# KadAMRN/Data_Free_Quantization

Measured on AMD Instinct MI355X. Metric: weight-GB/s quantized (per-ch INT8 DFQ sweep) + top-1 delta, MobileNetV2, higher is better.
Workload: dtype f32

## Files before the change

data_free_quantization_amd/csrc/dfq_cle.hip:

```cpp
#include "dfq_cle_common.h"

#include <algorithm>
#include <atomic>
#include <chrono>
#include <cmath>
#include <cstdio>
#include <cstdlib>
#include <cstring>
#include <condition_variable>
#include <functional>
#include <list>
#include <memory>
#include <mutex>
#include <thread>
#include <unordered_map>
#include <new>
#include <numeric>
#include <vector>

using namespace dfq;

namespace dfq {

struct CleRel {
    float* w1;
    float* w2;
    float* b1;
    float* bnw;
    float* bnb;
    float* sacc;
    int64_t c1, len1, o2, i2, khw2, o2g;
    int64_t moff;
    int32_t sacc_init;
    int32_t vec1;
    int32_t vec2;
    int32_t fuse_next;
    int32_t dw_prev;
    int32_t w1_self;
    int32_t w2_self;
};

enum : int32_t { kRangeW1 = 0, kRangeW2Contig = 1, kRangeW2Tile = 2, kRangeReset = 3, kRangeResetW1 = 4 };
enum : int32_t { kApplyW1 = 0, kApplyW2Contig = 1, kApplyW2Tile = 2, kApplyChannels = 3, kApplyDwBoth = 4 };

struct CleTask {
    int32_t rel;
    int32_t kind;
    int64_t a, b;
    int64_t c0, c1;
};

struct CleLayer {
    float* w;
    float* snap;
    int64_t n;
    int64_t nt;
};

struct CleChunk {
    int32_t layer;
    int32_t t;
    int64_t c0;
    int64_t len;
};

struct CleState {
    double diff;
    double thr;
    int32_t iter_count;
    int32_t iters;
    int32_t done;
    int32_t count;
    int32_t max_iters;
    int32_t error;
};

constexpr int kCleW1RowsPerTask = 4;
constexpr int kCleW2ChansPerTask = 4;

__host__ __device__ inline int row_group_lanes(int64_t len) {
    if (len >= 64) return 64;
    int g = 1;
    while (g < len) g <<= 1;
    return g;
}
__host__ __device__ inline int64_t rows_per_task(int64_t len) { return 4 * (64 / row_group_lanes(len)); }

__device__ __forceinline__ float group_min(float v, int g) {
    for (int off = g >> 1; off >= 1; off >>= 1) v = fminf(v, __shfl_xor(v, off, 64));
    return v;
}
__device__ __forceinline__ float group_max(float v, int g) {
    for (int off = g >> 1; off >= 1; off >>= 1) v = fmaxf(v, __shfl_xor(v, off, 64));
    return v;
}
template <class F>
__device__ __forceinline__ void for_short_rows(int64_t a, int64_t b, int64_t len, F&& f) {
    const int lane = threadIdx.x & 63, wv = threadIdx.x >> 6;
    const int G = row_group_lanes(len), rpw = 64 / G;
    const int sub = lane / G, sl = lane % G;
    for (int64_t base = a + (int64_t)wv * rpw; base < b; base += (int64_t)(kThreads / 64) * rpw) {
        const int64_t c = base + sub;
        f(c, c < b, sl, G);
    }
}
constexpr int64_t kCleChansPerTask = 1024;
constexpr int64_t kCleW1SmallElems = 2048, kCleDwRowsMult = 1;

__device__ __forceinline__ void wave_range(const float* __restrict__ p_, int64_t n, bool vec, int lane, float& vmin,
                                           float& vmax) {
    const DFQ_GLOBAL float* __restrict__ p = (const DFQ_GLOBAL float*)p_;
    vmin = INFINITY;
    vmax = -INFINITY;
    if (vec) {
        const DFQ_GLOBAL f32x4* p4 = (const DFQ_GLOBAL f32x4*)p;
        const int64_t n4 = n >> 2;
        for (int64_t i = lane; i < n4; i += 4 * 64) {
            f32x4 v[4];
#pragma unroll
            for (int u = 0; u < 4; ++u)
                if (i + 64 * u < n4) v[u] = p4[i + 64 * u];
#pragma unroll
            for (int u = 0; u < 4; ++u)
                if (i + 64 * u < n4) {
                    vmin = fminf(vmin, fminf(fminf(v[u].x, v[u].y), fminf(v[u].z, v[u].w)));
                    vmax = fmaxf(vmax, fmaxf(fmaxf(v[u].x, v[u].y), fmaxf(v[u].z, v[u].w)));
                }
        }
    } else {
        for (int64_t i = lane; i < n; i += 4 * 64) {
            float v[4];
#pragma unroll
            for (int u = 0; u < 4; ++u)
                if (i + 64 * u < n) v[u] = p[i + 64 * u];
#pragma unroll
            for (int u = 0; u < 4; ++u)
                if (i + 64 * u < n) {
                    vmin = fminf(vmin, v[u]);
                    vmax = fmaxf(vmax, v[u]);
                }
        }
    }
    cle_wave_minmax(vmin, vmax);
}

template <class F>
__device__ __forceinline__ void wave_scale(float* __restrict__ p_, int64_t n, bool vec, int lane, F&& factor) {
    DFQ_GLOBAL float* __restrict__ p = (DFQ_GLOBAL float*)p_;
    float f = 0.f;
    bool have = false;
    if (vec) {
        DFQ_GLOBAL f32x4* p4 = (DFQ_GLOBAL f32x4*)p;
        const int64_t n4 = n >> 2;
        for (int64_t i = lane; i < n4; i += 4 * 64) {
            f32x4 v[4];
#pragma unroll
            for (int u = 0; u < 4; ++u)
                if (i + 64 * u < n4) v[u] = p4[i + 64 * u];
            if (!have) {
                f = factor();
                have = true;
            }
#pragma unroll
            for (int u = 0; u < 4; ++u)
                if (i + 64 * u < n4) {
                    v[u].x = v[u].x * f;
                    v[u].y = v[u].y * f;
                    v[u].z = v[u].z * f;
                    v[u].w = v[u].w * f;
                    p4[i + 64 * u] = v[u];
                }
        }
    } else {
        for (int64_t i = lane; i < n; i += 4 * 64) {
            float v[4];
#pragma unroll
            for (int u = 0; u < 4; ++u)
                if (i + 64 * u < n) v[u] = p[i + 64 * u];
            if (!have) {
                f = factor();
                have = true;
            }
#pragma unroll
            for (int u = 0; u < 4; ++u)
                if (i + 64 * u < n) p[i + 64 * u] = v[u] * f;
        }
    }
}

template <class F>
__device__ __forceinline__ void wave_scale_mm(float* __restrict__ p_, int64_t n, bool vec, int lane, float& vmin,
                                              float& vmax, F&& factor) {
    DFQ_GLOBAL float* __restrict__ p = (DFQ_GLOBAL float*)p_;
    vmin = INFINITY;
    vmax = -INFINITY;
    float f = 0.f;
    bool have = false;
    if (vec) {
        DFQ_GLOBAL f32x4* p4 = (DFQ_GLOBAL f32x4*)p;
        const int64_t n4 = n >> 2;
        for (int64_t i = lane; i < n4; i += 4 * 64) {
            f32x4 v[4];
#pragma unroll
            for (int u = 0; u < 4; ++u)
                if (i + 64 * u < n4) v[u] = p4[i + 64 * u];
            if (!have) {
                f = factor();
                have = true;
            }
#pragma unroll
            for (int u = 0; u < 4; ++u)
                if (i + 64 * u < n4) {
                    v[u].x = v[u].x * f;
                    v[u].y = v[u].y * f;
                    v[u].z = v[u].z * f;
                    v[u].w = v[u].w * f;
                    p4[i + 64 * u] = v[u];
                    vmin = fminf(vmin, fminf(fminf(v[u].x, v[u].y), fminf(v[u].z, v[u].w)));
                    vmax = fmaxf(vmax, fmaxf(fmaxf(v[u].x, v[u].y), fmaxf(v[u].z, v[u].w)));
                }
        }
    } else {
        for (int64_t i = lane; i < n; i += 4 * 64) {
            float v[4];
#pragma unroll
            for (int u = 0; u < 4; ++u)
                if (i + 64 * u < n) v[u] = p[i + 64 * u];
            if (!have) {
                f = factor();
                have = true;
            }
#pragma unroll
            for (int u = 0; u < 4; ++u)
                if (i + 64 * u < n) {
                    const float y = v[u] * f;
                    p[i + 64 * u] = y;
                    vmin = fminf(vmin, y);
                    vmax = fmaxf(vmax, y);
                }
        }
    }
    cle_wave_minmax(vmin, vmax);
}

template <class F>
__device__ __forceinline__ void wave_scale_range(float* __restrict__ p_, int64_t n, int lane, float& vmin, float& vmax,
                                                 F&& factor) {
    DFQ_GLOBAL float* __restrict__ p = (DFQ_GLOBAL float*)p_;
    vmin = INFINITY;
    vmax = -INFINITY;
    float f = 0.f;
    bool have = false;
    for (int64_t i = lane; i < n; i += 64) {
        const float x = p[i];
        if (!have) {
            f = factor();
            have = true;
        }
        const float y = x * f;
        p[i] = y;
        vmin = fminf(vmin, y);
        vmax = fmaxf(vmax, y);
    }
    cle_wave_minmax(vmin, vmax);
}

constexpr int kTileMaxKhw = 9;
#ifndef DFQ_CLE_POS_ROWS
#define DFQ_CLE_POS_ROWS 4
#endif
constexpr int kPosTileMaxRows = DFQ_CLE_POS_ROWS;

__device__ __forceinline__ bool tile_by_position(const CleRel& R, const CleTask& tk) {
    return R.khw2 > 1 && R.khw2 <= kTileMaxKhw && (tk.a / R.o2g) == ((tk.b - 1) / R.o2g);
}

__device__ void tile_range_by_position(const CleRel& R, const CleTask& tk, uint32_t* __restrict__ mn,
                                       uint32_t* __restrict__ mx, float* __restrict__ tl) {
    const int t = threadIdx.x;
    const int khw = (int)R.khw2;
    const int64_t rowlen = R.i2 * R.khw2;
    const int ncol = (int)(tk.c1 - tk.c0);
    const int npos = ncol * khw;
    const DFQ_GLOBAL float* base = (const DFQ_GLOBAL float*)(R.w2 + tk.c0 * R.khw2);
    float vmn[kTileMaxKhw], vmx[kTileMaxKhw];
#pragma unroll
    for (int m = 0; m < kTileMaxKhw; ++m) {
        vmn[m] = INFINITY;
        vmx[m] = -INFINITY;
    }
    for (int64_t o = tk.a; o < tk.b; ++o) {
        const DFQ_GLOBAL float* rp = base + o * rowlen;
        float v[kTileMaxKhw];
#pragma unroll
        for (int m = 0; m < kTileMaxKhw; ++m)
            if (m < khw && t + kThreads * m < npos) v[m] = rp[t + kThreads * m];
#pragma unroll
        for (int m = 0; m < kTileMaxKhw; ++m)
            if (m < khw && t + kThreads * m < npos) {
                vmn[m] = fminf(vmn[m], v[m]);
                vmx[m] = fmaxf(vmx[m], v[m]);
            }
    }
#pragma unroll
    for (int m = 0; m < kTileMaxKhw; ++m)
        if (m < khw && t + kThreads * m < npos) {
            tl[t + kThreads * m] = vmn[m];
            tl[kThreads * kTileMaxKhw + t + kThreads * m] = vmx[m];
        }
    __syncthreads();
    if (t < ncol) {
        float a = INFINITY, b = -INFINITY;
        for (int k = 0; k < khw; ++k) {
            a = fminf(a, tl[t * khw + k]);
            b = fmaxf(b, tl[kThreads * kTileMaxKhw + t * khw + k]);
        }
        const int64_t c = R.c1 + (tk.a / R.o2g) * R.i2 + tk.c0 + t;
        atomicMin(&mn[c], enc_ord(a));
        atomicMax(&mx[c], enc_ord(b));
    }
    __syncthreads();
}

__device__ __forceinline__ void cle_range_body(const CleRel* __restrict__ rels, const CleTask* __restrict__ tasks,
                                               int64_t t0, int64_t t1, uint32_t* __restrict__ rng, int64_t M, int par,
                                               int64_t blk, int64_t nblk, float* tl) {
    uint32_t* mins = rng + (int64_t)par * 2 * M;
    uint32_t* maxs = mins + M;
    uint32_t* omins = rng + (int64_t)(par ^ 1) * 2 * M;
    uint32_t* omaxs = omins + M;
    const int lane = threadIdx.x & 63;
    const int wv = threadIdx.x >> 6;
    for (int64_t t = t0 + blk; t < t1; t += nblk) {
        const CleTask tk = tasks[t];
        const CleRel& R = rels[tk.rel];
        uint32_t* mn = mins + R.moff;
        uint32_t* mx = maxs + R.moff;
        if (tk.kind == kRangeW1 && R.len1 < 64) {
            for_short_rows(tk.a, tk.b, R.len1, [&](int64_t c, bool act, int sl, int G) {
                float vmin = INFINITY, vmax = -INFINITY;
                if (act)
                    for (int64_t i = sl; i < R.len1; i += G) {
                        const float x = ((DFQ_GLOBAL float*)R.w1)[c * R.len1 + i];
                        vmin = fminf(vmin, x);
                        vmax = fmaxf(vmax, x);
                    }
                vmin = group_min(vmin, G);
                vmax = group_max(vmax, G);
                if (act && sl == 0) {
                    mn[c] = enc_ord(vmin);
                    mx[c] = enc_ord(vmax);
                }
            });
        } else if (tk.kind == kRangeW2Contig && R.o2g * R.khw2 < 64) {
            const int64_t seg = R.o2g * R.khw2;
            for_short_rows(tk.a, tk.b, seg, [&](int64_t c, bool act, int sl, int G) {
                float vmin = INFINITY, vmax = -INFINITY;
                if (act)
                    for (int64_t i = sl; i < seg; i += G) {
                        const float x = ((DFQ_GLOBAL float*)R.w2)[c * seg + i];
                        vmin = fminf(vmin, x);
                        vmax = fmaxf(vmax, x);
                    }
                vmin = group_min(vmin, G);
                vmax = group_max(vmax, G);
                if (act && sl == 0) {
                    mn[R.c1 + c] = enc_ord(vmin);
                    mx[R.c1 + c] = enc_ord(vmax);
                }
            });
        } else if (tk.kind == kRangeW1) {
            for (int64_t c = tk.a + wv; c < tk.b; c += kThreads / 64) {
                float vmin, vmax;
                wave_range(R.w1 + c * R.len1, R.len1, R.vec1, lane, vmin, vmax);
                if (lane == 0) {
                    mn[c] = enc_ord(vmin);
                    mx[c] = enc_ord(vmax);
                }
            }
        } else if (tk.kind == kRangeW2Contig) {
            const int64_t seg = R.o2g * R.khw2;
            for (int64_t c = tk.a + wv; c < tk.b; c += kThreads / 64) {
                float vmin, vmax;
                wave_range(R.w2 + c * seg, seg, R.vec2, lane, vmin, vmax);
                if (lane == 0) {
                    mn[R.c1 + c] = enc_ord(vmin);
                    mx[R.c1 + c] = enc_ord(vmax);
                }
            }
        } else if (tk.kind == kRangeW2Tile) {
            if (tile_by_position(R, tk)) {
                tile_range_by_position(R, tk, mn, mx, tl);
                continue;
            }
            const int64_t rowlen = R.i2 * R.khw2;
            const bool one_group = (tk.a / R.o2g) == ((tk.b - 1) / R.o2g);
            for (int64_t i = tk.c0 + threadIdx.x; i < tk.c1; i += kThreads) {
                float vmin = INFINITY, vmax = -INFINITY;
                if (one_group && R.khw2 == 1) {
                    float v[kColTileRows];
#pragma unroll
                    for (int j = 0; j < kColTileRows; ++j)
                        if (tk.a + j < tk.b) v[j] = ((DFQ_GLOBAL float*)R.w2)[(tk.a + j) * rowlen + i];
#pragma unroll
                    for (int j = 0; j < kColTileRows; ++j)
                        if (tk.a + j < tk.b) {
                            vmin = fminf(vmin, v[j]);
                            vmax = fmaxf(vmax, v[j]);
                        }
                    const int64_t c = R.c1 + (tk.a / R.o2g) * R.i2 + i;
                    atomicMin(&mn[c], enc_ord(vmin));
                    atomicMax(&mx[c], enc_ord(vmax));
                    continue;
                }
                int64_t g_prev = -1;
                for (int64_t o = tk.a; o < tk.b; ++o) {
                    const int64_t g = o / R.o2g;
                    if (g != g_prev && g_prev >= 0) {
                        atomicMin(&mn[R.c1 + g_prev * R.i2 + i], enc_ord(vmin));
                        atomicMax(&mx[R.c1 + g_prev * R.i2 + i], enc_ord(vmax));
                        vmin = INFINITY;
                        vmax = -INFINITY;
                    }
                    g_prev = g;
                    const DFQ_GLOBAL float* p = (const DFQ_GLOBAL float*)(R.w2 + o * rowlen + i * R.khw2);
                    for (int64_t k = 0; k < R.khw2; ++k) {
                        vmin = fminf(vmin, p[k]);
                        vmax = fmaxf(vmax, p[k]);
                    }
                }
                if (g_prev >= 0) {
                    atomicMin(&mn[R.c1 + g_prev * R.i2 + i], enc_ord(vmin));
                    atomicMax(&mx[R.c1 + g_prev * R.i2 + i], enc_ord(vmax));
                }
            }
        } else {
            const int64_t off = R.moff + (tk.kind == kRangeReset ? R.c1 : 0);
            for (int64_t c = tk.a + threadIdx.x; c < tk.b; c += kThreads) {
                omins[off + c] = 0xFFFFFFFFu;
                omaxs[off + c] = 0u;
            }
        }
    }
}

__global__ void __launch_bounds__(kThreads)
cle_loop_range_kernel(const CleRel* __restrict__ rels, const CleTask* __restrict__ tasks, int64_t t0, int64_t t1,
                      uint32_t* __restrict__ rng, int64_t M, const CleState* __restrict__ st, int next) {
    __shared__ float tl[2 * kThreads * kTileMaxKhw];
    if (st->done) return;
    cle_range_body(rels, tasks, t0, t1, rng, M, (st->iters + next) & 1, blockIdx.x, gridDim.x, tl);
}

__device__ __forceinline__ CleScale cle_rel_scale(const CleRel* __restrict__ rels, const CleRel& R,
                                                  const uint32_t* __restrict__ mins, const uint32_t* __restrict__ maxs,
                                                  int64_t c, int is_signed, float eps, double smin, double smax) {
    if (R.dw_prev < 0) return cle_scale(mins + R.moff, maxs + R.moff, R.c1, c, is_signed, eps, smin, smax);
    const CleRel& Q = rels[R.dw_prev];
    const CleScale q = cle_scale(mins + Q.moff, maxs + Q.moff, Q.c1, c, is_signed, eps, smin, smax);
    const float mn1 = dec_ord(mins[Q.moff + Q.c1 + c]) * q.inv;
    const float mx1 = dec_ord(maxs[Q.moff + Q.c1 + c]) * q.inv;
    return cle_scale_from(mn1, mx1, dec_ord(mins[R.moff + R.c1 + c]), dec_ord(maxs[R.moff + R.c1 + c]), is_signed, eps,
                          smin, smax);
}

struct CleApplyLds {
    float red[2][kThreads / 64][kColTileRows];
    float inv_s[kThreads];
    float inv_pos[kThreads * kTileMaxKhw];
    float rows[kColTileRows * kThreads];
};

#ifdef DFQ_DIAGNOSTICS
__device__ uint64_t* g_cle_tl = nullptr;
__device__ uint64_t* g_cle_tl2 = nullptr;
__device__ int64_t g_cle_tl2_a0 = -1;
constexpr int kCleTl2Fin = 8192;
#endif

template <bool POS = true>
__device__ __forceinline__ void cle_apply_body(const CleRel* __restrict__ rels, const CleTask* __restrict__ tasks,
                                               int64_t t0, int64_t t1, uint32_t* __restrict__ rng, int64_t M,
                                               int par, bool first_iter, int is_signed, float eps, double smin,
                                               double smax, int64_t blk, int64_t nblk, CleApplyLds& A,
                                               float* __restrict__ vsave = nullptr, int32_t* __restrict__ vtag = nullptr,
                                               int32_t iter = 0) {
    auto& red = A.red;
    float* rows = A.rows;
    float* inv_s = A.inv_s;
    float* inv_pos = A.inv_pos;
    uint32_t* mins = rng + (int64_t)par * 2 * M;
    uint32_t* maxs = mins + M;
    uint32_t* nmins = rng + (int64_t)(par ^ 1) * 2 * M;
    uint32_t* nmaxs = nmins + M;
    const int lane = threadIdx.x & 63;
    const int wv = threadIdx.x >> 6;
    for (int64_t t = t0 + blk; t < t1; t += nblk) {
#ifdef DFQ_DIAGNOSTICS
        const bool tl_on = g_cle_tl != nullptr;
        const uint64_t tl_start = tl_on ? __builtin_amdgcn_s_memrealtime() : 0;
        uint64_t tl_sub = 0;
#define DFQ_CLE_TL_MARK(k) \
        if (tl_on) tl_sub |= (1ull << 63) | (((__builtin_amdgcn_s_memrealtime() - tl_start) & 0xffffull) << (16 * (k)));
#else
#define DFQ_CLE_TL_MARK(k)
#endif
        const CleTask tk = tasks[t];
        const CleRel& R = rels[tk.rel];
        const uint32_t* mn = mins + R.moff;
        const uint32_t* mx = maxs + R.moff;
        if (tk.kind == kApplyW1 && R.len1 < 64) {
            for_short_rows(tk.a, tk.b, R.len1, [&](int64_t c, bool act, int sl, int G) {
                float y0 = INFINITY, y1 = -INFINITY;
                if (act && sl < R.len1) {
                    DFQ_GLOBAL float* p = (DFQ_GLOBAL float*)(R.w1 + c * R.len1 + sl);
                    const float x = *p;
                    const float y = x * cle_rel_scale(rels, R, mins, maxs, c, is_signed, eps, smin, smax).s;
                    *p = y;
                    y0 = y1 = y;
                }
                if (R.w1_self) {
                    y0 = group_min(y0, G);
                    y1 = group_max(y1, G);
                    if (act && sl == 0) {
                        nmins[R.moff + c] = enc_ord(y0);
                        nmaxs[R.moff + c] = enc_ord(y1);
                    }
                }
            });
        } else if (tk.kind == kApplyDwBoth && R.o2g * R.khw2 < 64) {
            const CleRel& N = rels[tk.c0];
            const int64_t seg = R.o2g * R.khw2;
            for_short_rows(tk.a, tk.b, seg, [&](int64_t c, bool act, int sl, int G) {
                float z0 = INFINITY, z1 = -INFINITY;
                if (act && sl < seg) {
                    DFQ_GLOBAL float* p = (DFQ_GLOBAL float*)(R.w2 + c * seg + sl);
                    const float x = *p;
                    const float inv = cle_rel_scale(rels, R, mins, maxs, c, is_signed, eps, smin, smax).inv;
                    const float sn = cle_rel_scale(rels, N, mins, maxs, c, is_signed, eps, smin, smax).s;
                    const float y = x * inv;
                    const float z = y * sn;
                    *p = z;
                    z0 = z1 = z;
                }
                if (R.w2_self) {
                    z0 = group_min(z0, G);
                    z1 = group_max(z1, G);
                    if (act && sl == 0) {
                        nmins[R.moff + R.c1 + c] = enc_ord(z0);
                        nmaxs[R.moff + R.c1 + c] = enc_ord(z1);
                    }
                }
            });
        } else if (tk.kind == kApplyW2Contig && R.o2g * R.khw2 < 64) {
            const int64_t seg = R.o2g * R.khw2;
            const bool fuse = R.fuse_next >= 0;
            for_short_rows(tk.a, tk.b, seg, [&](int64_t c, bool act, int sl, int G) {
                float vmin = INFINITY, vmax = -INFINITY;
                if (act && sl < seg) {
                    DFQ_GLOBAL float* p = (DFQ_GLOBAL float*)(R.w2 + c * seg + sl);
                    const float x = *p;
                    const float y = x * cle_rel_scale(rels, R, mins, maxs, c, is_signed, eps, smin, smax).inv;
                    *p = y;
                    vmin = vmax = y;
                }
                if (fuse) {
                    vmin = group_min(vmin, G);
                    vmax = group_max(vmax, G);
                    if (act && sl == 0) {
                        const int64_t off = rels[R.fuse_next].moff;
                        mins[off + c] = enc_ord(vmin);
                        maxs[off + c] = enc_ord(vmax);
                    }
                }
            });
        } else if (tk.kind == kApplyW1) {
            for (int64_t c = tk.a + wv; c < tk.b; c += kThreads / 64) {
                auto sc = [&] { return cle_rel_scale(rels, R, mins, maxs, c, is_signed, eps, smin, smax).s; };
                if (R.w1_self) {
                    float y0, y1;
                    wave_scale_mm(R.w1 + c * R.len1, R.len1, R.vec1, lane, y0, y1, sc);
                    if (lane == 0) {
                        nmins[R.moff + c] = enc_ord(y0);
                        nmaxs[R.moff + c] = enc_ord(y1);
                    }
                } else {
                    wave_scale(R.w1 + c * R.len1, R.len1, R.vec1, lane, sc);
                }
            }
        } else if (tk.kind == kApplyDwBoth) {
            const CleRel& N = rels[tk.c0];
            const int64_t seg = R.o2g * R.khw2;
            for (int64_t c = tk.a + wv; c < tk.b; c += kThreads / 64) {
                const float inv = cle_rel_scale(rels, R, mins, maxs, c, is_signed, eps, smin, smax).inv;
                const float sn = cle_rel_scale(rels, N, mins, maxs, c, is_signed, eps, smin, smax).s;
                DFQ_GLOBAL float* p = (DFQ_GLOBAL float*)(R.w2 + c * seg);
                float z0 = INFINITY, z1 = -INFINITY;
                for (int64_t i = lane; i < seg; i += 64) {
                    const float y = p[i] * inv;
                    const float z = y * sn;
                    p[i] = z;
                    z0 = fminf(z0, z);
                    z1 = fmaxf(z1, z);
                }
                if (R.w2_self) {
                    cle_wave_minmax(z0, z1);
                    if (lane == 0) {
                        nmins[R.moff + R.c1 + c] = enc_ord(z0);
                        nmaxs[R.moff + R.c1 + c] = enc_ord(z1);
                    }
                }
            }
        } else if (tk.kind == kApplyW2Contig) {
            const int64_t seg = R.o2g * R.khw2;
            for (int64_t c = tk.a + wv; c < tk.b; c += kThreads / 64) {
                auto inv = [&] { return cle_rel_scale(rels, R, mins, maxs, c, is_signed, eps, smin, smax).inv; };
                if (R.fuse_next >= 0) {
                    float vmin, vmax;
                    wave_scale_range(R.w2 + c * seg, seg, lane, vmin, vmax, inv);
                    if (lane == 0) {
                        const int64_t off = rels[R.fuse_next].moff;
                        mins[off + c] = enc_ord(vmin);
                        maxs[off + c] = enc_ord(vmax);
                    }
                } else {
                    wave_scale(R.w2 + c * seg, seg, R.vec2, lane, inv);
                }
            }
        } else if (POS && tk.kind == kApplyW2Tile && tile_by_position(R, tk) && tk.b - tk.a <= kPosTileMaxRows) {
            const int t = threadIdx.x;
            const int khw = (int)R.khw2;
            const int64_t rowlen = R.i2 * R.khw2;
            const int ncol = (int)(tk.c1 - tk.c0);
            const int npos = ncol * khw;
            DFQ_GLOBAL float* base = (DFQ_GLOBAL float*)(R.w2 + tk.c0 * R.khw2);
            const bool fuse = R.fuse_next >= 0;
            if (t < ncol)
                inv_s[t] = cle_rel_scale(rels, R, mins, maxs, (tk.a / R.o2g) * R.i2 + tk.c0 + t, is_signed, eps, smin, smax).inv;
            __syncthreads();
            DFQ_CLE_TL_MARK(0)
            for (int q = t; q < npos; q += kThreads) inv_pos[q] = inv_s[q / khw];
            __syncthreads();
            DFQ_CLE_TL_MARK(1)
            float v[kPosTileMaxRows][kTileMaxKhw];
#pragma unroll
            for (int r = 0; r < kPosTileMaxRows; ++r) {
                const DFQ_GLOBAL float* rb = base + (tk.a + r) * rowlen;
#pragma unroll
                for (int m = 0; m < kTileMaxKhw; ++m)
                    if (tk.a + r < tk.b && m < khw && t + kThreads * m < npos) v[r][m] = rb[t + kThreads * m];
            }
#pragma unroll
            for (int r = 0; r < kPosTileMaxRows; ++r) {
                if (tk.a + r >= tk.b) break;
                DFQ_GLOBAL float* rp = base + (tk.a + r) * rowlen;
                float lo = INFINITY, hi = -INFINITY;
#pragma unroll
                for (int m = 0; m < kTileMaxKhw; ++m)
                    if (m < khw && t + kThreads * m < npos) {
                        const float y = v[r][m] * inv_pos[t + kThreads * m];
                        rp[t + kThreads * m] = y;
                        lo = fminf(lo, y);
                        hi = fmaxf(hi, y);
                    }
                if (fuse) {
                    cle_wave_minmax(lo, hi);
                    if (lane == 0) {
                        red[0][wv][r] = lo;
                        red[1][wv][r] = hi;
                    }
                }
            }
            __syncthreads();
            DFQ_CLE_TL_MARK(2)
            if (fuse && t < tk.b - tk.a) {
                float a = red[0][0][t], b = red[1][0][t];
                for (int w = 1; w < kThreads / 64; ++w) {
                    a = fminf(a, red[0][w][t]);
                    b = fmaxf(b, red[1][w][t]);
                }
                const int64_t off = rels[R.fuse_next].moff + tk.a + t;
                atomicMin(&mins[off], enc_ord(a));
                atomicMax(&maxs[off], enc_ord(b));
            }
            __syncthreads();
        } else if (tk.kind == kApplyW2Tile && R.fuse_next >= 0) {
            const int64_t rowlen = R.i2 * R.khw2;
            const int64_t i = tk.c0 + threadIdx.x;
            const bool act = i < tk.c1;
            const bool one_group = (tk.a / R.o2g) == ((tk.b - 1) / R.o2g);
            const int nr = (int)(tk.b - tk.a);
            if (one_group && R.khw2 == 1) {
                float v[kColTileRows];
#pragma unroll
                for (int j = 0; j < kColTileRows; ++j)
                    if (act && j < nr) v[j] = ((DFQ_GLOBAL float*)R.w2)[(tk.a + j) * rowlen + i];
                const float inv =
                    act ? cle_rel_scale(rels, R, mins, maxs, (tk.a / R.o2g) * R.i2 + i, is_signed, eps, smin, smax).inv : 0.f;
#pragma unroll
                for (int j = 0; j < kColTileRows; ++j) {
                    if (j < nr) {
                        float y = __builtin_nanf("");
                        if (act) {
                            y = v[j] * inv;
                            ((DFQ_GLOBAL float*)R.w2)[(tk.a + j) * rowlen + i] = y;
                        }
                        rows[j * kThreads + threadIdx.x] = y;
                    }
                    if (j == 0) {
                        DFQ_CLE_TL_MARK(0)
                    }
                }
                DFQ_CLE_TL_MARK(1)
                block_lds_sync();
                const int r = threadIdx.x >> 4, sg = threadIdx.x & 15;
                float lo = INFINITY, hi = -INFINITY;
                if (r < nr) {
                    const float4* q = reinterpret_cast<const float4*>(rows + r * kThreads + sg * 16);
#pragma unroll
                    for (int u = 0; u < 4; ++u) {
                        const float4 x = q[u];
                        lo = fminf(lo, fminf(fminf(x.x, x.y), fminf(x.z, x.w)));
                        hi = fmaxf(hi, fmaxf(fmaxf(x.x, x.y), fmaxf(x.z, x.w)));
                    }
                }
                lo = fminf(lo, dpp_f(lo, 0xB1));
                hi = fmaxf(hi, dpp_f(hi, 0xB1));
                lo = fminf(lo, dpp_f(lo, 0x4E));
                hi = fmaxf(hi, dpp_f(hi, 0x4E));
                lo = fminf(lo, dpp_f(lo, 0x141));
                hi = fmaxf(hi, dpp_f(hi, 0x141));
                lo = fminf(lo, dpp_f(lo, 0x140));
                hi = fmaxf(hi, dpp_f(hi, 0x140));
                DFQ_CLE_TL_MARK(2)
                if (sg == 0 && r < nr) {
                    const int64_t off = rels[R.fuse_next].moff + tk.a + r;
                    atomicMin(&mins[off], enc_ord(lo));
                    atomicMax(&maxs[off], enc_ord(hi));
                }
            } else {
                int64_t g_prev = -1;
                float inv = 0.f;
                for (int j = 0; j < nr; ++j) {
                    const int64_t o = tk.a + j;
                    float lo = INFINITY, hi = -INFINITY;
                    if (act) {
                        const int64_t g = o / R.o2g;
                        if (g != g_prev) {
                            inv = cle_rel_scale(rels, R, mins, maxs, g * R.i2 + i, is_signed, eps, smin, smax).inv;
                            g_prev = g;
                        }
                        DFQ_GLOBAL float* p = (DFQ_GLOBAL float*)(R.w2 + o * rowlen + i * R.khw2);
                        for (int64_t k = 0; k < R.khw2; ++k) {
                            const float y = p[k] * inv;
                            p[k] = y;
                            lo = fminf(lo, y);
                            hi = fmaxf(hi, y);
                        }
                    }
                    float a = lo, b = hi;
                    cle_wave_minmax(a, b);
                    if (lane == 0) {
                        red[0][wv][j] = a;
                        red[1][wv][j] = b;
                    }
                }
                __syncthreads();
                if (threadIdx.x < tk.b - tk.a) {
                    const int j = threadIdx.x;
                    float a = red[0][0][j], b = red[1][0][j];
                    for (int w = 1; w < kThreads / 64; ++w) {
                        a = fminf(a, red[0][w][j]);
                        b = fmaxf(b, red[1][w][j]);
                    }
                    const int64_t off = rels[R.fuse_next].moff + tk.a + j;
                    atomicMin(&mins[off], enc_ord(a));
                    atomicMax(&maxs[off], enc_ord(b));
                }
            }
            __syncthreads();
        } else if (tk.kind == kApplyW2Tile) {
            const int64_t rowlen = R.i2 * R.khw2;
            const bool one_group = (tk.a / R.o2g) == ((tk.b - 1) / R.o2g);
            for (int64_t i = tk.c0 + threadIdx.x; i < tk.c1; i += kThreads) {
                if (one_group && R.khw2 == 1) {
                    float v[kColTileRows];
#pragma unroll
                    for (int j = 0; j < kColTileRows; ++j)
                        if (tk.a + j < tk.b) v[j] = ((DFQ_GLOBAL float*)R.w2)[(tk.a + j) * rowlen + i];
                    const float inv = cle_rel_scale(rels, R, mins, maxs, (tk.a / R.o2g) * R.i2 + i, is_signed, eps, smin,
                                                smax).inv;
                    ((DFQ_GLOBAL float*)R.w2)[tk.a * rowlen + i] = v[0] * inv;
                    DFQ_CLE_TL_MARK(0)
#pragma unroll
                    for (int j = 1; j < kColTileRows; ++j)
                        if (tk.a + j < tk.b) ((DFQ_GLOBAL float*)R.w2)[(tk.a + j) * rowlen + i] = v[j] * inv;
                    DFQ_CLE_TL_MARK(1)
                    continue;
                }
                int64_t g_prev = -1;
                float inv = 0.f;
                for (int64_t o = tk.a; o < tk.b; ++o) {
                    const int64_t g = o / R.o2g;
                    if (g != g_prev) {
                        inv = cle_rel_scale(rels, R, mins, maxs, g * R.i2 + i, is_signed, eps, smin, smax).inv;
                        g_prev = g;
                    }
                    DFQ_GLOBAL float* p = (DFQ_GLOBAL float*)(R.w2 + o * rowlen + i * R.khw2);
                    for (int64_t k = 0; k < R.khw2; ++k) p[k] = p[k] * inv;
                }
            }
        } else {
            if (vtag && threadIdx.x == 0) vtag[t] = iter;
            for (int64_t c = tk.a + threadIdx.x; c < tk.b; c += kThreads) {
                const CleScale cs = cle_rel_scale(rels, R, mins, maxs, c, is_signed, eps, smin, smax);
                if (vsave) {
                    float* v = vsave + 2 * R.moff;
                    if (R.b1) v[c] = R.b1[c];
                    if (R.bnw) v[R.c1 + c] = R.bnw[c];
                    if (R.bnb) v[2 * R.c1 + c] = R.bnb[c];
                    if (R.sacc) v[3 * R.c1 + c] = R.sacc[c];
                }
                if (R.b1) R.b1[c] = R.b1[c] * cs.s;
                if (R.bnw) R.bnw[c] = R.bnw[c] * cs.s;
                if (R.bnb) R.bnb[c] = R.bnb[c] * cs.s;
                if (R.sacc) R.sacc[c] = (R.sacc_init && first_iter) ? cs.s : R.sacc[c] * cs.s;
            }
        }
#ifdef DFQ_DIAGNOSTICS
        if (tl_on) {
            __syncthreads();
            if (threadIdx.x == 0) {
                uint32_t hw, xcc;
                asm volatile("s_getreg_b32 %0, hwreg(HW_REG_HW_ID)" : "=s"(hw));
                asm volatile("s_getreg_b32 %0, hwreg(HW_REG_XCC_ID)" : "=s"(xcc));
                uint64_t* r = g_cle_tl + 4 * t;
                r[0] = tl_start;
                r[1] = __builtin_amdgcn_s_memrealtime();
                r[2] = tl_sub ? tl_sub : (((uint64_t)xcc << 32) | hw);
                r[3] = (uint64_t)tk.kind | ((uint64_t)tk.rel << 8) | ((uint64_t)(tk.b - tk.a) << 24);
            }
        }
#endif
    }
}

constexpr int kCleTile = 8192;
constexpr int kCleTailWords = 64;

struct CleUnit {
    int32_t chunk;
    int32_t tile;
};

__global__ void __launch_bounds__(kThreads)
cle_loop_init_kernel(const CleLayer* __restrict__ layers, const CleChunk* __restrict__ chunks, int64_t nchunks,
                     const CleUnit* __restrict__ units, int64_t nunits, uint32_t* __restrict__ rng, int64_t M,
                     float* __restrict__ part, int64_t npart, uint32_t* __restrict__ cnt, int64_t ncnt,
                     int32_t* __restrict__ vtag, int64_t nvtag, CleState* __restrict__ st, CleState init) {
    const int64_t gt = (int64_t)blockIdx.x * kThreads + threadIdx.x, gs = (int64_t)gridDim.x * kThreads;
    for (int64_t i = gt; i < 4 * M; i += gs) rng[i] = ((i / M) & 1) ? 0u : 0xFFFFFFFFu;
    for (int64_t i = gt; i < npart; i += gs) part[i] = 0.f;
    for (int64_t i = gt; i < ncnt; i += gs) cnt[i] = 0u;
    for (int64_t i = gt; i < nvtag; i += gs) vtag[i] = -1;
    if (gt == 0) *st = init;
    for (int64_t u = blockIdx.x; u < nunits; u += gridDim.x) {
        const CleUnit un = units[u];
        const CleChunk ch = chunks[un.chunk];
        const CleLayer Ly = layers[ch.layer];
        const int64_t nb1 = (ch.len / 32) / 256;
        const int64_t e0 = (int64_t)un.tile * 8192;
        const int64_t e1 = un.tile < nb1 ? e0 + 8192 : ch.len;
        for (int64_t i = e0 + threadIdx.x; i < e1; i += kThreads) Ly.snap[ch.c0 + i] = Ly.w[ch.c0 + i];
    }
    if (blockIdx.x == 0)
        for (int64_t k = 0; k < nchunks; ++k) {
            const CleChunk ch = chunks[k];
            if (ch.len >= 8) continue;
            const CleLayer Ly = layers[ch.layer];
            for (int64_t i = threadIdx.x; i < ch.len; i += kThreads) Ly.snap[ch.c0 + i] = Ly.w[ch.c0 + i];
        }
}


struct CleNoUnitHook {
    __device__ void operator()(const CleUnit&, const CleChunk&, int64_t) const {}
};

template <class Hook = CleNoUnitHook>
__device__ __forceinline__ void cle_tiles_body(const CleLayer* __restrict__ layers, const CleChunk* __restrict__ chunks,
                                               const int64_t* __restrict__ b1off, const CleUnit* __restrict__ units,
                                               int64_t nunits, float* __restrict__ b1buf, float* __restrict__ tailbuf,
                                               int64_t blk, int64_t nblk, float* d, float* b0, Hook hook = Hook()) {
    const int tid = threadIdx.x;
    for (int64_t u = blk; u < nunits; u += nblk) {
        const CleUnit un = units[u];
        const CleChunk ch = chunks[un.chunk];
        const CleLayer Ly = layers[ch.layer];
        const DFQ_GLOBAL float* __restrict__ w = (const DFQ_GLOBAL float*)(Ly.w + ch.c0);
        DFQ_GLOBAL float* __restrict__ sn = (DFQ_GLOBAL float*)(Ly.snap + ch.c0);
        const int64_t len = ch.len, sz = len / 32, vs = len / 8;
        const int64_t nb1 = sz / 256;
        const bool full = un.tile < nb1;
        const int64_t e0 = (int64_t)un.tile * kCleTile;
        const int64_t cnt = full ? kCleTile : len - e0;
        if (full) {
            float xs[2][16], ys[2][16];
#pragma unroll
            for (int h = 0; h < 2; ++h) {
                const int q = tid + h * kThreads;
                const int64_t base = e0 + 32 * (16 * (q >> 5)) + (q & 31);
#pragma unroll
                for (int j = 0; j < 16; ++j) {
                    xs[h][j] = w[base + 32 * j];
                    ys[h][j] = sn[base + 32 * j];
                }
            }
#pragma unroll
            for (int h = 0; h < 2; ++h) {
                const int q = tid + h * kThreads;
                const int64_t base = e0 + 32 * (16 * (q >> 5)) + (q & 31);
                float a = 0.f;
#pragma unroll
                for (int j = 0; j < 16; ++j) {
                    a += fabsf(xs[h][j] - ys[h][j]);
                    sn[base + 32 * j] = xs[h][j];
                }
                b0[q] = a;
            }
            __syncthreads();
            if (tid < 32) {
                float a = 0.f;
#pragma unroll
                for (int m = 0; m < 16; ++m) a += b0[m * 32 + tid];
                st_coh(b1buf + b1off[un.chunk] + (int64_t)un.tile * 32 + tid, a);
            }
        } else {
            for (int64_t e = tid; e < cnt; e += 8 * kThreads) {
                float x[8], y[8];
#pragma unroll
                for (int u = 0; u < 8; ++u)
                    if (e + u * kThreads < cnt) {
                        x[u] = w[e0 + e + u * kThreads];
                        y[u] = sn[e0 + e + u * kThreads];
                    }
#pragma unroll
                for (int u = 0; u < 8; ++u)
                    if (e + u * kThreads < cnt) {
                        d[e + u * kThreads] = fabsf(x[u] - y[u]);
                        sn[e0 + e + u * kThreads] = x[u];
                    }
            }
            __syncthreads();
            const int64_t ni = sz - nb1 * 256;
            const int64_t rem_b0 = ni / 16, tail0 = ni % 16;
            float* tb = tailbuf + (int64_t)un.chunk * kCleTailWords;
            if (tid < 32) {
                float a1p = 0.f;
                for (int64_t m = 0; m < rem_b0; ++m) {
                    float a = 0.f;
                    for (int j = 0; j < 16; ++j) a += d[32 * (16 * m + j) + tid];
                    a1p += a;
                }
                float a0t = 0.f;
                for (int64_t j = 0; j < tail0; ++j) a0t += d[32 * (16 * rem_b0 + j) + tid];
                float p = a0t;
                p += a1p;
                st_coh(tb + tid, p);
            } else if (tid < 64) {
                const int t = tid - 32;
                const int64_t nv = vs - 4 * sz;
                if (t < 24 && t < nv * 8) st_coh(tb + 32 + t, d[8 * (4 * sz) + t - e0]);
                if (t < 8 && t < len - 8 * vs) st_coh(tb + 56 + t, d[8 * vs + t - e0]);
            }
        }
        __syncthreads();
        hook(un, ch, nb1);
    }
}

constexpr int kCleTilesLds = kCleTile + kCleTailWords + 512;
constexpr int kCleRangeLds = 2 * kThreads * kTileMaxKhw;

template <class LdB1, class LdTb>
__device__ __forceinline__ float cle_chunk_sum_with(const CleChunk& ch, LdB1&& b1, LdTb&& tb, int lane) {
    const int64_t len = ch.len;
    const int64_t sz = len / 32, vs = len / 8;
    const int64_t nb1 = sz / 256, nb2 = nb1 / 16, rem_b1 = nb1 % 16;
    float fa = 0.f;
    float p = 0.f;
    if (lane < 32) {
        float a3 = 0.f;
        for (int64_t r = 0; r < nb2; ++r) {
            float b2 = 0.f;
            for (int q = 0; q < 16; ++q) b2 += b1((r * 16 + q) * 32 + lane);
            a3 += b2;
        }
        float a2p = 0.f;
        for (int64_t q = 0; q < rem_b1; ++q) a2p += b1((nb2 * 16 + q) * 32 + lane);
        p = tb(lane);
        p += a2p;
        p += a3;
    }
    auto ps = [&](int s) { return rl_f(p, s); };
    for (int64_t e = 0; e < len - 8 * vs; ++e) fa += tb(56 + e);
    const int64_t nv = vs - 4 * sz;
    for (int l = 0; l < 8; ++l) {
        float p0 = ps(l);
        for (int64_t v = 0; v < nv; ++v) p0 += tb(32 + v * 8 + l);
        p0 += ps(l + 8);
        p0 += ps(l + 16);
        p0 += ps(l + 24);
        fa += p0;
    }
    return fa;
}

__device__ __forceinline__ float cle_chunk_sum(const CleChunk& ch, const float* b1, const float* tb, int lane) {
    const DFQ_GLOBAL float* g1 = (const DFQ_GLOBAL float*)b1;
    const DFQ_GLOBAL float* gt = (const DFQ_GLOBAL float*)tb;
    return cle_chunk_sum_with(ch, [g1](int64_t i) { return ld_coh(g1 + i); }, [gt](int64_t i) { return ld_coh(gt + i); },
                              lane);
}

__device__ __forceinline__ float cle_tiny_chunk_sum(const CleLayer* __restrict__ layers, const CleChunk& ch) {
    const CleLayer Ly = layers[ch.layer];
    float* w = Ly.w + ch.c0;
    float* sn = Ly.snap + ch.c0;
    return aten_inner_sum([&](int64_t e) {
        const float x = w[e];
        const float dd = fabsf(x - sn[e]);
        sn[e] = x;
        return dd;
    }, ch.len);
}

template <class P>
__device__ __forceinline__ double np_pairwise_leaf(P x, int64_t n) {
    if (n < 8) {
        double res = 0.;
        for (int64_t i = 0; i < n; ++i) res += x[i];
        return res;
    }
    double r[8];
#pragma unroll
    for (int j = 0; j < 8; ++j) r[j] = x[j];
    int64_t i;
    for (i = 8; i < n - (n % 8); i += 8)
#pragma unroll
        for (int j = 0; j < 8; ++j) r[j] += x[i + j];
    double res = ((r[0] + r[1]) + (r[2] + r[3])) + ((r[4] + r[5]) + (r[6] + r[7]));
    for (; i < n; ++i) res += x[i];
    return res;
}

struct NpFrame {
    int64_t o, n;
    int64_t state;
};
constexpr int kNpFrames = 48;
constexpr int kNpStackFloats = kNpFrames * (int)(sizeof(NpFrame) + sizeof(double)) / 4;
template <class P>
__device__ double np_pairwise(P a, int64_t n, float* stack) {
    if (n <= 128) return 0. + np_pairwise_leaf(a, n);
    NpFrame* fr = reinterpret_cast<NpFrame*>(stack);
    double* acc = reinterpret_cast<double*>(fr + kNpFrames);
    int fp = 0, ap = 0;
    fr[fp++] = {0, n, 0};
    while (fp > 0) {
        NpFrame& f = fr[fp - 1];
        if (f.n <= 128) {
            acc[ap++] = np_pairwise_leaf(a + f.o, f.n);
            --fp;
        } else if (f.state == 0) {
            int64_t n2 = f.n / 2;
            n2 -= n2 % 8;
            f.state = 1;
            const NpFrame left{f.o, n2, 0}, right{f.o + n2, f.n - n2, 0};
            fr[fp++] = right;
            fr[fp++] = left;
        } else {
            const double right = acc[--ap];
            const double left = acc[--ap];
            acc[ap++] = left + right;
            --fp;
        }
    }
    return 0. + acc[0];
}

template <bool kLeafOnly = false, bool kCoherent = false>
__device__ __forceinline__ void cle_final_body(const CleLayer* __restrict__ layers, int32_t nl,
                                               const float* __restrict__ part, int32_t S, double* __restrict__ means,
                                               double* __restrict__ hist, CleState* __restrict__ st, double* sm,
                                               float* part_lds = nullptr, float* np_stack = nullptr,
                                               uint32_t* hflag = nullptr) {
#ifdef DFQ_DIAGNOSTICS
    uint64_t* tlm = (kCoherent && threadIdx.x == 0 && g_cle_tl2) ? g_cle_tl2 + 4 * kCleTl2Fin : nullptr;
#endif
    constexpr int kStateWords = (int)(sizeof(CleState) / 4);
    static_assert(sizeof(CleState) % 4 == 0, "CleState: whole 4-B words");
    const int64_t nps = (int64_t)nl * (S + 2);
    DFQ_LDS float* pls = (DFQ_LDS float*)part_lds;
    if (part_lds) {
        for (int64_t i = threadIdx.x; i < nps + kStateWords; i += blockDim.x) {
            const DFQ_GLOBAL float* src = (const DFQ_GLOBAL float*)(i < nps ? part + i
                                                                           : reinterpret_cast<const float*>(st) + (i - nps));
            pls[i] = kCoherent ? ld_coh(src) : *src;
        }
        __syncthreads();
    }
#ifdef DFQ_DIAGNOSTICS
    if (tlm) tlm[2] = __builtin_amdgcn_s_memrealtime();
#endif
    DFQ_LDS double* ms = (DFQ_LDS double*)sm;
    DFQ_GLOBAL double* mg = (DFQ_GLOBAL double*)means;
    const bool m_lds = nl <= 1024;
    double* m = m_lds ? sm : means;
    for (int l = threadIdx.x; l < nl; l += blockDim.x) {
        const float* pl = (part_lds ? part_lds : part) + (int64_t)l * S;
        auto ld = [&](int64_t e) { return (part_lds || !kCoherent) ? pl[e] : ld_coh(pl + e); };
        const float* lm = part_lds ? part_lds + (int64_t)nl * S + 2 * l : nullptr;
        const bool serial = lm ? lm[1] != 0.f : layers[l].nt == 1;
        const float sum = serial ? 0.f + (0.f + ld(0)) : 0.f + aten_inner_sum([&](int64_t e) { return ld(e); }, S);
        m[l] = (double)(sum / (lm ? lm[0] : (float)layers[l].n));
    }
    __syncthreads();
#ifdef DFQ_DIAGNOSTICS
    if (tlm) tlm[3] = __builtin_amdgcn_s_memrealtime();
#endif
    if (threadIdx.x == 0) {
        CleState s0;
        if (part_lds) {
            __builtin_memcpy(&s0, part_lds + nps, sizeof(CleState));
        } else {
            s0 = *st;
        }
        double dt = 0.0;
        if constexpr (kLeafOnly) {
            dt = nl > 0 ? 0. + (m_lds ? np_pairwise_leaf(ms, nl) : np_pairwise_leaf(mg, nl)) : 0.0;
        } else {
            dt = nl > 0 ? (m_lds ? np_pairwise(ms, nl, np_stack) : np_pairwise(mg, nl, np_stack)) : 0.0;
        }
        const int it = s0.iters;
        hist[it] = dt;
        int ic = s0.iter_count;
        double diff = s0.diff;
        if (fabs(diff - dt) > 1e-9) {
            ic = 0;
            diff = dt;
        } else {
            ic += 1;
        }
        const bool cont = (diff > s0.thr) && (ic < s0.count);
        const int done = (!cont || it + 1 >= s0.max_iters) ? 1 : 0;
        st->iters = it + 1;
        st->iter_count = ic;
        st->diff = diff;
        st->done = done;
        if (hflag)
            __hip_atomic_store(hflag, ((uint32_t)(it + 1) << 1) | (uint32_t)done, __ATOMIC_RELAXED,
                               __HIP_MEMORY_SCOPE_SYSTEM);
    }
}

__device__ __forceinline__ bool handoff_arrive(uint32_t* c, uint32_t target) {
    return __hip_atomic_fetch_add(c, 1u, __ATOMIC_RELAXED, __HIP_MEMORY_SCOPE_AGENT) == target;
}

__host__ __device__ inline int64_t cle_stop_blocks(int64_t nchunks) {
    return nchunks > 0 ? (nchunks + kThreads / 64 - 1) / (kThreads / 64) : 1;
}

struct CleFin {
    uint32_t* cnt;
    float* part;
    double* means;
    double* hist;
    int64_t nchunks, nbig;
    int32_t S, nl;
    int32_t last;
    uint32_t* hflag;
    int32_t stop_arrival;
};

static_assert(kCleTilesLds - kCleTile >= kNpStackFloats, "np_pairwise's frame stack after the tile area");
union CleStepLds {
    CleApplyLds apply;
    float tiles[kCleTilesLds > kCleRangeLds ? kCleTilesLds : kCleRangeLds];
};

constexpr bool kCleTilesFirst = true;
#ifdef DFQ_DIAGNOSTICS
__device__ int g_cle_tiles_first = kCleTilesFirst ? 1 : 0;
#endif

template <bool POS>
#ifndef DFQ_CLE_POS_WAVES
#define DFQ_CLE_POS_WAVES 1
#endif
__global__ void __launch_bounds__(kThreads) __attribute__((amdgpu_waves_per_eu(POS ? DFQ_CLE_POS_WAVES : 4)))
cle_loop_step_kernel(const CleRel* __restrict__ rels, const CleTask* __restrict__ atasks, int64_t a0, int64_t a1,
                     int64_t nab, uint32_t* __restrict__ rng, int64_t M, int is_signed, float eps, double smin,
                     double smax, const CleLayer* __restrict__ layers, const CleChunk* __restrict__ chunks,
                     const int64_t* __restrict__ b1off, const CleUnit* __restrict__ units, int64_t uo, int64_t nuo,
                     int64_t nto, int64_t up, int64_t nup, int64_t ntp, float* __restrict__ b1buf,
                     float* __restrict__ tailbuf, const CleTask* __restrict__ rtasks, int64_t ro, int64_t nro_t,
                     int64_t nro, int64_t rp, int64_t nrp_t, int64_t nrp, CleFin F, CleState* __restrict__ st,
                     int32_t g, float* __restrict__ vsave, int32_t* __restrict__ vtag, int32_t stop_it) {
    __shared__ CleStepLds L;
    __shared__ int flag;
    if (st->done) return;
    int64_t blk = blockIdx.x;
#ifdef DFQ_DIAGNOSTICS
    const bool tiles_first = g_cle_tiles_first != 0;
#else
    constexpr bool tiles_first = kCleTilesFirst;
#endif
    const int64_t nstop = stop_it >= 0 ? cle_stop_blocks(F.nchunks) : 0;
    if (tiles_first) {
        const int64_t ns = nab + nstop, ntl = nto + ntp;
        if (blk < ntl) blk += ns;
        else if (blk < ntl + ns) blk -= ntl;
    }
    if (blk < nab) {
        cle_apply_body<POS>(rels, atasks, a0, a1, rng, M, g & 1, g == 0, is_signed, eps, smin, smax, blk, nab, L.apply,
                            vsave, vtag, g);
        return;
    }
    blk -= nab;
#ifdef DFQ_DIAGNOSTICS
    const bool tl2 = g_cle_tl2 != nullptr && blk < kCleTl2Fin && (g_cle_tl2_a0 < 0 || (a0 == g_cle_tl2_a0 && nab > 0));
    const uint64_t tl2_start = tl2 ? __builtin_amdgcn_s_memrealtime() : 0;
    auto tl2_rec = [&](int role) {
        if (tl2 && threadIdx.x == 0) {
            uint64_t* r = g_cle_tl2 + 4 * blk;
            r[0] = tl2_start;
            r[1] = __builtin_amdgcn_s_memrealtime();
            r[2] = (uint64_t)role;
        }
    };
#else
    auto tl2_rec = [](int) {};
#endif
    float* lds = L.tiles;
    auto finish = [&]() {
#ifdef DFQ_DIAGNOSTICS
        const uint64_t tf0 = __builtin_amdgcn_s_memrealtime();
#endif
        if (threadIdx.x == 0 && F.nchunks > F.nbig)
            for (int64_t k = 0; k < F.nchunks; ++k) {
                const CleChunk c2 = chunks[k];
                if (c2.len < 8) st_coh(F.part + (int64_t)c2.layer * F.S + c2.t, 0.f + cle_tiny_chunk_sum(layers, c2));
            }
        asm volatile("s_waitcnt vmcnt(0)" ::: "memory");
        __syncthreads();
        const bool stage_part = (int64_t)F.nl * (F.S + 2) + (int64_t)(sizeof(CleState) / 4) + 2048 <= kCleTile;
        if (F.nl <= 128)
            cle_final_body<true, true>(layers, F.nl, F.part, F.S, F.means, F.hist, st, reinterpret_cast<double*>(lds),
                                       stage_part ? lds + 2048 : nullptr, nullptr, F.hflag);
        else
            cle_final_body<false, true>(layers, F.nl, F.part, F.S, F.means, F.hist, st,
                                        reinterpret_cast<double*>(lds), stage_part ? lds + 2048 : nullptr,
                                        lds + kCleTile, F.hflag);
#ifdef DFQ_DIAGNOSTICS
        if (tl2 && threadIdx.x == 0) {
            uint64_t* r = g_cle_tl2 + 4 * kCleTl2Fin;
            r[0] = tf0;
            r[1] = __builtin_amdgcn_s_memrealtime();
        }
#endif
    };
    if (stop_it >= 0) {
        if (blk < nstop) {
            const int64_t c = blk * (kThreads / 64) + (threadIdx.x >> 6);
            if (c < F.nchunks) {
                const CleChunk ch = chunks[c];
                if (ch.len >= 8) {
                    const float fa = cle_chunk_sum(ch, b1buf + b1off[c], tailbuf + c * kCleTailWords, threadIdx.x & 63);
                    if ((threadIdx.x & 63) == 0) st_coh(F.part + (int64_t)ch.layer * F.S + ch.t, 0.f + fa);
                }
            }
            asm volatile("s_waitcnt vmcnt(0)" ::: "memory");
            __syncthreads();
            if (threadIdx.x == 0)
                flag = handoff_arrive(F.cnt + F.nchunks, ((uint32_t)stop_it + 1u) * (uint32_t)nstop - 1u);
            __syncthreads();
            if (flag) finish();
            return;
        }
        blk -= nstop;
    }
    const int64_t ntiles = nto + ntp;
    if (blk >= ntiles) {
        blk -= ntiles;
        const bool own = blk < nro;
        const int64_t b = own ? blk : blk - nro;
        cle_range_body(rels, rtasks, own ? ro : rp, (own ? ro : rp) + (own ? nro_t : nrp_t), rng, M,
                       own ? (g + 1) & 1 : g & 1, b, own ? nro : nrp, L.tiles);
        tl2_rec(2);
        return;
    }
    const bool own = blk < nto;
    const int32_t it = own ? g : g - 1;
    const int64_t tb = own ? blk : blk - nto;
    const int64_t tnb = own ? nto : ntp;
    const uint32_t round = (uint32_t)it + 1u;
    auto arrive = [&](uint32_t* c, uint32_t members) -> bool {
        asm volatile("s_waitcnt vmcnt(0)" ::: "memory");
        __syncthreads();
        if (threadIdx.x == 0) flag = handoff_arrive(c, round * members - 1u);
        __syncthreads();
        return flag != 0;
    };
    if (F.nbig == 0) {
        if (own && tb == 0 && F.last) finish();
        return;
    }
    const uint32_t fin_members = (uint32_t)F.nbig;
    auto hook = [&](const CleUnit& un, const CleChunk& ch, int64_t nb1) {
        if (!arrive(F.cnt + un.chunk, (uint32_t)(nb1 + 1))) return;
        {
            const float* gb1 = b1buf + b1off[un.chunk];
            const float* gtb = tailbuf + (int64_t)un.chunk * kCleTailWords;
            const int64_t nw = 32 * nb1;
            const bool staged = nw + kCleTailWords <= kCleTile;
            if (staged) {
                DFQ_LDS float* ll = (DFQ_LDS float*)lds;
                const DFQ_GLOBAL float* g1 = (const DFQ_GLOBAL float*)gb1;
                for (int64_t i = threadIdx.x; i < nw; i += kThreads) ll[i] = ld_coh(g1 + i);
                if (threadIdx.x < kCleTailWords) ll[nw + threadIdx.x] = ld_coh((const DFQ_GLOBAL float*)gtb + threadIdx.x);
            }
            __syncthreads();
            if (threadIdx.x < 64) {
                const float fa = staged ? cle_chunk_sum_with(ch, [&](int64_t i) { return lds[i]; },
                                                             [&](int64_t i) { return lds[nw + i]; }, threadIdx.x)
                                        : cle_chunk_sum(ch, gb1, gtb, threadIdx.x);
                if (threadIdx.x == 0) st_coh(F.part + (int64_t)ch.layer * F.S + ch.t, 0.f + fa);
            }
        }
        if (F.stop_arrival && arrive(F.cnt + F.nchunks, fin_members)) finish();
    };
    if (F.stop_arrival)
        cle_tiles_body<decltype(hook)>(layers, chunks, b1off, units + (own ? uo : up), own ? nuo : nup, b1buf, tailbuf,
                                       tb, tnb, lds, lds + kCleTile + kCleTailWords, hook);
    else
        cle_tiles_body(layers, chunks, b1off, units + (own ? uo : up), own ? nuo : nup, b1buf, tailbuf, tb, tnb, lds,
                       lds + kCleTile + kCleTailWords);
#ifdef DFQ_DIAGNOSTICS
    if (tl2) {
        const CleUnit un0 = units[(own ? uo : up) + tb];
        tl2_rec(un0.tile >= (chunks[un0.chunk].len / 32) / 256 ? 3 : 1);
    }
#else
    tl2_rec(1);
#endif
}

__global__ void __launch_bounds__(kThreads)
cle_loop_rollback_kernel(const CleLayer* __restrict__ layers, int32_t nl, const CleRel* __restrict__ rels,
                         const CleTask* __restrict__ atasks, int64_t n_at, const float* __restrict__ vsave,
                         const int32_t* __restrict__ vtag, const CleState* __restrict__ st) {
    const int32_t A = st->iters;
    const int64_t gt = (int64_t)blockIdx.x * kThreads + threadIdx.x, gs = (int64_t)gridDim.x * kThreads;
    for (int32_t l = 0; l < nl; ++l) {
        const CleLayer Ly = layers[l];
        for (int64_t i = gt; i < Ly.n; i += gs) Ly.w[i] = Ly.snap[i];
    }
    for (int64_t t = blockIdx.x; t < n_at; t += gridDim.x) {
        const CleTask tk = atasks[t];
        if (tk.kind != kApplyChannels || vtag[t] != A) continue;
        const CleRel& R = rels[tk.rel];
        const float* v = vsave + 2 * R.moff;
        for (int64_t c = tk.a + threadIdx.x; c < tk.b; c += kThreads) {
            if (R.b1) R.b1[c] = v[c];
            if (R.bnw) R.bnw[c] = v[R.c1 + c];
            if (R.bnb) R.bnb[c] = v[2 * R.c1 + c];
            if (R.sacc) R.sacc[c] = v[3 * R.c1 + c];
        }
    }
}

}

constexpr int32_t kCleHistCap = 1025;

struct dfq_cle_plan {
    CleRel* d_rels = nullptr;
    CleTask* d_rtasks = nullptr;
    CleTask* d_atasks = nullptr;
    CleLayer* d_layers = nullptr;
    CleChunk* d_chunks = nullptr;
    uint32_t* d_rng = nullptr;
    float* d_part = nullptr;
    int32_t slots = 8;
    double* d_means = nullptr;
    double* d_hist = nullptr;
    double* d_hist_tables = nullptr;
    CleState* d_state = nullptr;
    CleState* h_state = nullptr;
    uint32_t* d_flag = nullptr;
    uint64_t* d_sig = nullptr;
    uint64_t gen = 0;
    hipStream_t st = nullptr;
    std::vector<int64_t> rstep, astep;
    std::vector<char> step_pos;
    int64_t M = 0, nchunks = 0;
    int32_t nl = 0, chains = 0, steps = 0;
    bool fused = false;
    CleUnit* d_units = nullptr;
    int64_t* d_b1off = nullptr;
    float* d_b1 = nullptr;
    float* d_tail = nullptr;
    int64_t nunits = 0;
    double smin = 1e-8, smax = 1e8;
    int32_t is_signed = 0;
    float eps = 0.f;
    void* d_tables = nullptr;
    bool pooled = false;
    void* d_snap_owned = nullptr;
    uint32_t* d_cnt = nullptr;
    int64_t nbig = 0;
    int64_t ri0 = 0, ri1 = 0;
    std::vector<int64_t> uoffs, roffs;
    int32_t nlaunch = 0;
    int32_t stop_off = -1;
    bool lagged = false;
    float* d_vsave = nullptr;
    int32_t* d_vtag = nullptr;
    int64_t n_at = 0;
    int dev = 0;
    struct CleAsync* async = nullptr;
    bool abandoned = false;
    int64_t bytes[3] = {0, 0, 0};
    bool timed = false;
    float loop_ms = -1.f;
    int32_t launched = 0;
#ifdef DFQ_DIAGNOSTICS
    std::vector<CleRel> h_rels;
    std::vector<CleTask> h_atasks;
#endif
};

static bool cle_timing() {
    static const bool on = ab_env("DFQ_CLE_TIMING") != nullptr;
    return on;
}
static double now_us() {
    return std::chrono::duration<double, std::micro>(std::chrono::steady_clock::now().time_since_epoch()).count();
}

struct CleDeviceCtx {
    std::mutex mu;
    hipStream_t st = nullptr;
    CleState* h_state = nullptr;
    uint32_t* h_flag = nullptr;
    uint32_t* d_flag = nullptr;
    char* d_pool = nullptr;
    size_t pool_cap = 0;
    char* h_pool = nullptr;
    size_t hpool_cap = 0;
    bool pool_busy = false;
    uint64_t pool_struct = 0;
    hipEvent_t pool_ev = nullptr;
    double* d_hist = nullptr;
    int64_t hist_cap = 0;
    double* h_hist = nullptr;
    int64_t h_hist_cap = 0;
    void* sig = nullptr;
    int sig_state = 0;
    uint64_t gen = 0;
    struct dfq_cle_plan* pending = nullptr;
    hipEvent_t in_ev = nullptr;
    struct CleWorker* worker = nullptr;
};
static CleDeviceCtx& cle_device_ctx(int dev) {
    static CleDeviceCtx ctx[64];
    return ctx[dev & 63];
}
static hipError_t cle_ctx_ready(CleDeviceCtx& ctx) {
    hipError_t e = hipSuccess;
    if (!ctx.st) {
        int least = 0, greatest = 0;
        e = hipDeviceGetStreamPriorityRange(&least, &greatest);
        if (e == hipSuccess) e = hipStreamCreateWithPriority(&ctx.st, hipStreamNonBlocking, greatest);
    }
    if (e == hipSuccess && !ctx.h_state) e = hipHostMalloc(&ctx.h_state, sizeof(CleState));
    if (e == hipSuccess && !ctx.h_flag) {
        e = hipHostMalloc(&ctx.h_flag, 64, hipHostMallocMapped | hipHostMallocCoherent);
        if (e == hipSuccess) e = hipHostGetDevicePointer(reinterpret_cast<void**>(&ctx.d_flag), ctx.h_flag, 0);
    }
    if (e == hipSuccess && !ctx.pool_ev) e = hipEventCreateWithFlags(&ctx.pool_ev, hipEventDisableTiming);
    if (e == hipSuccess && !ctx.in_ev) e = hipEventCreateWithFlags(&ctx.in_ev, hipEventDisableTiming);
    return e;
}

static void cle_plan_free(dfq_cle_plan* p) {
    const double t0 = now_us();
    if (p->pooled) {
        CleDeviceCtx& ctx = cle_device_ctx(p->dev);
        std::lock_guard<std::mutex> lock(ctx.mu);
        ctx.pool_busy = false;
    } else {
        (void)hipFree(p->d_tables);
    }
    (void)hipFree(p->d_snap_owned);
    if (cle_timing()) fprintf(stderr, "DFQ_CLE_TIMING free: %.1f us\n", now_us() - t0);
    delete p;
}

static int64_t snap_bytes(int64_t n) { return ceil_div(n * (int64_t)sizeof(float), (int64_t)256) * 256; }

struct TableLayout {
    int64_t total = 0;
    template <typename T>
    int64_t add(int64_t count) {
        const int64_t off = total;
        total += ceil_div((int64_t)sizeof(T) * std::max<int64_t>(count, 1), (int64_t)256) * 256;
        return off;
    }
};

extern "C" int64_t dfq_cle_plan_ws_bytes(const int64_t* target_n, int32_t n_targets) {
    if (n_targets < 0 || (n_targets > 0 && !target_n)) return -1;
    int64_t b = 0;
    for (int32_t l = 0; l < n_targets; ++l) {
        if (target_n[l] < 0) return -1;
        b += snap_bytes(target_n[l]);
    }
    return b;
}

struct CleStructure {
    std::vector<CleRel> R;
    int64_t M = 0;
    int32_t chains = 0, steps = 0;
    bool fused = false;
    std::vector<CleTask> rt, at;
    std::vector<int64_t> rstep, astep;
    int64_t ri0 = 0, ri1 = 0;
    std::vector<CleLayer> layers;
    std::vector<CleChunk> chunks;
    std::vector<CleUnit> units;
    std::vector<int64_t> b1off;
    int64_t nb1_total = 0;
    std::vector<int64_t> uoffs, roffs;
    int32_t nlaunch = 0, stop_off = -1;
    bool lagged = false;
    double t_chains = 0, t_tasks = 0, t_chunks = 0, t_place = 0;
    int64_t bytes_rescale = 0, bytes_metric = 0, bytes_range = 0;
    uint64_t id = 0;
};
static std::atomic<uint64_t> g_struct_ids{0};

static int cle_build_structure(std::vector<CleRel> R, int64_t M, int32_t n_rel, float* const* targets,
                               const int64_t* target_n, int32_t n_targets, int32_t ref_threads, CleStructure& S) {
    const double tp1 = now_us();
    std::vector<int32_t> parent(n_rel);
    std::iota(parent.begin(), parent.end(), 0);
    auto find = [&](int32_t x) {
        while (parent[x] != x) x = parent[x] = parent[parent[x]];
        return x;
    };
    for (int32_t a = 0; a < n_rel; ++a) {
        const void* pa[5] = {R[a].w1, R[a].w2, R[a].b1, R[a].bnw, R[a].bnb};
        for (int32_t b = 0; b < a; ++b) {
            const void* pb[5] = {R[b].w1, R[b].w2, R[b].b1, R[b].bnw, R[b].bnb};
            bool share = false;
            for (int i = 0; i < 5 && !share; ++i)
                for (int j = 0; j < 5 && !share; ++j) share = pa[i] && pa[i] == pb[j];
            if (share) parent[find(a)] = find(b);
        }
    }
    std::vector<int32_t> step_of(n_rel), comp_len(n_rel, 0);
    int32_t chains = 0, steps = 0;
    for (int32_t r = 0; r < n_rel; ++r) {
        const int32_t c = find(r);
        if (comp_len[c] == 0) ++chains;
        step_of[r] = comp_len[c]++;
        steps = std::max(steps, step_of[r] + 1);
    }
    std::vector<int32_t> w1_src(n_rel, -1);
    bool fused = true;
    {
        const char* fe = ab_env("DFQ_CLE_FUSED");
        if (fe && fe[0] == '0') fused = false;
        std::vector<std::vector<int32_t>> chain_of(n_rel);
        for (int32_t r = 0; r < n_rel; ++r) chain_of[find(r)].push_back(r);
        for (const auto& L : chain_of) {
            for (size_t j = 0; j < L.size() && fused; ++j) {
                const CleRel& cr = R[L[j]];
                for (size_t i = 0; i < j && fused; ++i) {
                    const CleRel& cq = R[L[i]];
                    if (cq.w1 == cr.w2 || cq.w2 == cr.w2) fused = false;
                    if (cq.w1 == cr.w1 || cq.w2 == cr.w1) {
                        const bool ok = i + 1 == j && cq.w2 == cr.w1 && cq.w1 != cr.w1 && w1_src[L[j]] < 0 &&
                                        (cq.i2 > 1 || cq.o2g == 1) && cr.c1 == cq.o2 && cr.len1 == cq.i2 * cq.khw2;
                        if (ok) w1_src[L[j]] = L[i];
                        else fused = false;
                    }
                }
            }
        }
        if (fused)
            for (int32_t r = 0; r < n_rel; ++r)
                if (w1_src[r] >= 0) R[w1_src[r]].fuse_next = r;
    }
    std::vector<int32_t> dw_next(n_rel, -1);
    if (fused) {
        for (int32_t r = 0; r < n_rel; ++r) {
            const int32_t q = w1_src[r];
            if (q < 0 || R[q].dw_prev >= 0 || dw_next[q] >= 0) continue;
            const CleRel& cq = R[q];
            const CleRel& cr = R[r];
            const bool dw = cq.i2 == 1 && cq.o2g == 1 && cq.o2 == cq.c1 && cr.c1 == cq.o2 && cr.len1 == cq.khw2;
            if (!dw) continue;
            R[r].dw_prev = q;
            R[q].fuse_next = -1;
            dw_next[q] = r;
        }
        std::vector<int32_t> cur(n_rel, 0);
        steps = 0;
        for (int32_t r = 0; r < n_rel; ++r) {
            const int32_t c = find(r);
            step_of[r] = R[r].dw_prev >= 0 ? step_of[R[r].dw_prev] : cur[c]++;
            steps = std::max(steps, step_of[r] + 1);
        }
    }
    const double tp2 = now_us();
    std::vector<CleTask> rt, at;
    std::vector<CleTask>* rout = &rt;
    std::vector<int64_t> rstep(1, 0), astep(1, 0);
    auto w2_range_tasks = [&](int32_t r) {
        const CleRel& c = R[r];
        if (c.i2 == 1) {
            const int64_t k = rows_per_task(c.o2g * c.khw2);
            for (int64_t a = 0; a < c.c1; a += k)
                rout->push_back({r, kRangeW2Contig, a, std::min<int64_t>(a + k, c.c1), 0, 0});
        } else {
            for (int64_t a = 0; a < c.o2; a += kColTileRows)
                for (int64_t i0 = 0; i0 < c.i2; i0 += kThreads)
                    rout->push_back({r, kRangeW2Tile, a, std::min<int64_t>(a + kColTileRows, c.o2), i0,
                                     std::min<int64_t>(i0 + kThreads, c.i2)});
            for (int64_t a = 0; a < c.c1; a += kCleChansPerTask)
                rout->push_back({r, kRangeReset, a, std::min<int64_t>(a + kCleChansPerTask, c.c1), 0, 0});
        }
    };
    auto w1_range_tasks = [&](int32_t r) {
        const CleRel& c = R[r];
        if (c.dw_prev >= 0) return;
        if (fused && w1_src[r] >= 0) {
            for (int64_t a = 0; a < c.c1; a += kCleChansPerTask)
                rout->push_back({r, kRangeResetW1, a, std::min<int64_t>(a + kCleChansPerTask, c.c1), 0, 0});
        } else {
            const int64_t k = rows_per_task(c.len1);
            for (int64_t a = 0; a < c.c1; a += k)
                rout->push_back({r, kRangeW1, a, std::min<int64_t>(a + k, c.c1), 0, 0});
        }
    };
    const int64_t w1_mult = [] {
        const char* e = ab_env("DFQ_CLE_W1_ROWS");
        return e && *e ? std::max<int64_t>(1, atoll(e)) : int64_t(0);
    }();
    auto w1_rows = [&](int64_t len1) {
        const int64_t k = rows_per_task(len1);
        if (w1_mult > 0) return w1_mult * k;
        return k * len1 < kCleW1SmallElems ? 2 * k : k;
    };
    const int64_t dw_mult = [] {
        const char* e = ab_env("DFQ_CLE_DW_ROWS");
        return e && *e ? std::max<int64_t>(1, atoll(e)) : kCleDwRowsMult;
    }();
    auto apply_tasks = [&](int32_t r, std::vector<CleTask>& out) {
        const CleRel& c = R[r];
        if (c.dw_prev < 0)
            for (int64_t a = 0, k = w1_rows(c.len1); a < c.c1; a += k)
                out.push_back({r, kApplyW1, a, std::min<int64_t>(a + k, c.c1), 0, 0});
        if (dw_next[r] >= 0) {
            for (int64_t a = 0, k = dw_mult * rows_per_task(c.o2g * c.khw2); a < c.c1; a += k)
                out.push_back({r, kApplyDwBoth, a, std::min<int64_t>(a + k, c.c1), dw_next[r], 0});
        } else if (c.i2 == 1) {
            for (int64_t a = 0, k = rows_per_task(c.o2g * c.khw2); a < c.c1; a += k)
                out.push_back({r, kApplyW2Contig, a, std::min<int64_t>(a + k, c.c1), 0, 0});
        } else {
            const int64_t rows = (c.khw2 > 1 && c.khw2 <= kTileMaxKhw) ? kPosTileMaxRows : kColTileRows;
            for (int64_t a = 0; a < c.o2; a += rows)
                for (int64_t i0 = 0; i0 < c.i2; i0 += kThreads)
                    out.push_back({r, kApplyW2Tile, a, std::min<int64_t>(a + rows, c.o2), i0,
                                   std::min<int64_t>(i0 + kThreads, c.i2)});
        }
        for (int64_t a = 0; a < c.c1; a += kThreads)
            out.push_back({r, kApplyChannels, a, std::min<int64_t>(a + kThreads, c.c1), 0, 0});
    };
    int64_t ri0 = 0, ri1 = 0;
    if (fused) {
        for (int32_t r = 0; r < n_rel; ++r) {
            w1_range_tasks(r);
            w2_range_tasks(r);
        }
        rstep.push_back((int64_t)rt.size());
        for (int32_t r = 0; r < n_rel; ++r) {
            if (w1_src[r] < 0 && R[r].dw_prev < 0) R[r].w1_self = 1;
            if (dw_next[r] >= 0) R[r].w2_self = 1;
        }
        ri0 = (int64_t)rt.size();
        for (int64_t t = rstep[0]; t < rstep[1]; ++t) {
            const CleTask tk = rt[t];
            if (tk.kind == kRangeW1 && R[tk.rel].w1_self) continue;
            if (tk.kind == kRangeW2Contig && R[tk.rel].w2_self) continue;
            rt.push_back(tk);
        }
        ri1 = (int64_t)rt.size();
    }
    for (int32_t k = 0; k < steps; ++k) {
        for (int32_t r = 0; r < n_rel; ++r) {
            if (step_of[r] != k) continue;
            if (!fused) {
                w1_range_tasks(r);
                w2_range_tasks(r);
            }
            apply_tasks(r, at);
        }
        auto prio = [](int32_t kind) {
            switch (kind) {
                case kApplyW2Tile: return 0;
                case kApplyChannels: return 1;
                case kApplyDwBoth: return 2;
                case kApplyW1: return 3;
                default: return 4;
            }
        };
        std::stable_sort(at.begin() + astep.back(), at.end(),
                         [&](const CleTask& x, const CleTask& y) { return prio(x.kind) < prio(y.kind); });
        if (!fused) rstep.push_back((int64_t)rt.size());
        astep.push_back((int64_t)at.size());
    }
    const double tp3 = now_us();
    std::vector<CleLayer> layers(n_targets);
    std::vector<CleChunk> chunks;
    std::vector<CleUnit> units;
    std::vector<int64_t> b1off;
    int64_t nb1_total = 0;
    for (int32_t l = 0; l < n_targets; ++l) {
        const int64_t n = target_n[l];
        if (!targets[l] || n <= 0) return DFQ_ERR_INVALID;
        layers[l] = CleLayer{nullptr, nullptr, n, 1};
        int64_t nt = 1;
        if (n >= 32768 && ref_threads > 1) nt = std::min<int64_t>(ref_threads, ceil_div(n, (int64_t)32768));
        layers[l].nt = nt;
        const int64_t chunk = ceil_div(n, nt);
        for (int64_t t = 0; t < nt; ++t) {
            const int64_t b = t * chunk;
            if (b >= n) break;
            const int64_t len = std::min<int64_t>(n, b + chunk) - b;
            const int64_t sz = len / 32;
            if (aten_ceil_log2(sz) / 4 > 4) return DFQ_ERR_UNSUPPORTED;
            const int32_t ci = (int32_t)chunks.size();
            chunks.push_back(CleChunk{l, (int32_t)t, b, len});
            const int64_t nb1 = sz / 256;
            b1off.push_back(32 * nb1_total);
            nb1_total += nb1;
            if (len >= 8)
                for (int64_t g = 0; g <= nb1; ++g) units.push_back(CleUnit{ci, (int32_t)g});
        }
    }
    const double tp4 = now_us();
    const bool tiny = std::any_of(chunks.begin(), chunks.end(), [](const CleChunk& c) { return c.len < 8; });
    const bool have_tiles = std::any_of(chunks.begin(), chunks.end(), [](const CleChunk& c) { return c.len >= 8; });
    bool lag_ok = fused && !tiny && have_tiles && steps > 0;
    if (const char* e = ab_env("DFQ_CLE_LAG")) lag_ok = lag_ok && e[0] != '0';
    int32_t band_force = -1;
    const bool stop_arrival = [] {
        const char* e = ab_env("DFQ_CLE_STOP");
        return e && e[0] == 'a';
    }();
    if (const char* e = ab_env("DFQ_CLE_BAND")) band_force = atoi(e);
    std::vector<const float*> sp_w;
    std::vector<std::pair<int32_t, int32_t>> sp_v;
    auto sp_find = [&](const float* w) -> int32_t {
        for (size_t i = 0; i < sp_w.size(); ++i)
            if (sp_w[i] == w) return (int32_t)i;
        return -1;
    };
    std::vector<int32_t> rel_t1(n_rel), rel_t2(n_rel);
    for (int32_t r = 0; r < n_rel; ++r)
        for (int side = 0; side < 2; ++side) {
            const float* w = side ? R[r].w2 : R[r].w1;
            int32_t i = sp_find(w);
            if (i < 0) {
                i = (int32_t)sp_w.size();
                sp_w.push_back(w);
                sp_v.push_back({step_of[r], step_of[r]});
            } else {
                sp_v[i] = {std::min(sp_v[i].first, step_of[r]), std::max(sp_v[i].second, step_of[r])};
            }
            (side ? rel_t2 : rel_t1)[r] = i;
        }
    std::vector<int32_t> lay_t(n_targets);
    for (int32_t l = 0; l < n_targets; ++l) lay_t[l] = lag_ok ? sp_find(targets[l]) : -1;
    std::vector<int32_t> layer_off(n_targets, 0);
    int32_t stop_off = -1;
    std::vector<int32_t> rt_off;
    int32_t nlaunch = steps + 1;
    bool lagged = false;
    int32_t lag_max = -1;
    auto place = [&](int32_t nl_) -> bool {
        auto window = [&](int32_t ti) -> std::pair<int32_t, int32_t> {
            if (ti < 0) return {0, 2 * nl_ - 1};
            return {sp_v[ti].second + 1, std::min(2 * nl_ - 1, nl_ + sp_v[ti].first - 1)};
        };
        std::vector<double> base_load(nl_, 0.0);
        for (int32_t k = 0; k < steps && k < nl_; ++k)
            for (int64_t t = astep[k]; t < astep[k + 1]; ++t) {
                const CleTask& tk = at[t];
                const CleRel& q = R[tk.rel];
                double n = 0;
                if (tk.kind == kApplyW1) n = (double)(tk.b - tk.a) * q.len1;
                else if (tk.kind == kApplyW2Tile) n = (double)(tk.b - tk.a) * (tk.c1 - tk.c0) * q.khw2;
                else if (tk.kind != kApplyChannels) n = (double)(tk.b - tk.a) * q.o2g * q.khw2;
                base_load[k] += 8.0 * n;
            }
        const int64_t nr = ri1 - ri0;
        std::vector<std::pair<int32_t, int32_t>> rwin((size_t)nr);
        std::vector<double> rbytes((size_t)nr);
        for (int64_t x = 0; x < nr; ++x) {
            const CleTask& tk = rt[ri0 + x];
            const CleRel& q = R[tk.rel];
            std::pair<int32_t, int32_t> w;
            switch (tk.kind) {
                case kRangeW1:
                    w = window(rel_t1[tk.rel]);
                    rbytes[x] = 4.0 * (tk.b - tk.a) * q.len1;
                    break;
                case kRangeW2Contig:
                    w = window(rel_t2[tk.rel]);
                    rbytes[x] = 4.0 * (tk.b - tk.a) * q.o2g * q.khw2;
                    break;
                case kRangeW2Tile:
                    w = window(rel_t2[tk.rel]);
                    rbytes[x] = 4.0 * (tk.b - tk.a) * (tk.c1 - tk.c0) * q.khw2;
                    break;
                case kRangeReset:
                    w = {step_of[tk.rel] + 1, std::min(2 * nl_ - 1, nl_ + sp_v[rel_t2[tk.rel]].second)};
                    rbytes[x] = 64.0;
                    break;
                default:
                    w = {step_of[tk.rel] + 1, 2 * nl_ - 1};
                    rbytes[x] = 64.0;
            }
            if (w.first > w.second) return false;
            rwin[x] = w;
        }
        int32_t maxlo = 0, minhi = 2 * nl_ - 1;
        std::vector<std::pair<int32_t, int32_t>> lwin(n_targets);
        for (int32_t l = 0; l < n_targets; ++l) {
            lwin[l] = window(lay_t[l]);
            if (lwin[l].first > lwin[l].second) return false;
            maxlo = std::max(maxlo, lwin[l].first);
            minhi = std::min(minhi, lwin[l].second);
        }
        const int32_t bw = stop_arrival ? nl_ : nl_ - 1;
        if (bw < 1) return false;
        const int32_t b_lo = std::max(0, maxlo - bw + 1), b_hi = std::min(minhi, 2 * nl_ - 1 - bw);
        if (b_lo > b_hi) return false;
        std::vector<int32_t> lord(n_targets);
        std::iota(lord.begin(), lord.end(), 0);
        std::sort(lord.begin(), lord.end(),
                  [&](int32_t x, int32_t y) { return target_n[x] != target_n[y] ? target_n[x] > target_n[y] : x < y; });
        std::vector<int64_t> rord((size_t)nr);
        std::iota(rord.begin(), rord.end(), 0);
        std::sort(rord.begin(), rord.end(),
                  [&](int64_t x, int64_t y) { return rbytes[x] != rbytes[y] ? rbytes[x] > rbytes[y] : x < y; });
        double best = 1e300;
        std::vector<int32_t> roff((size_t)nr), loff(n_targets);
        for (int32_t B0 = b_lo; B0 <= b_hi; ++B0) {
            if (band_force >= 0 && B0 != band_force && band_force >= b_lo && band_force <= b_hi) continue;
            std::vector<double> load = base_load;
            auto pick = [&](int32_t lo, int32_t hi, double bytes) {
                int32_t bo = lo;
                for (int32_t o = lo; o <= hi; ++o)
                    if (load[o % nl_] < load[bo % nl_]) bo = o;
                load[bo % nl_] += bytes;
                return bo;
            };
            for (int64_t x : rord) roff[x] = pick(rwin[x].first, rwin[x].second, rbytes[x]);
            int32_t maxoff = 0;
            for (int32_t l : lord) {
                loff[l] = pick(std::max(lwin[l].first, B0), std::min(lwin[l].second, B0 + bw - 1), 12.0 * target_n[l]);
                maxoff = std::max(maxoff, loff[l]);
            }
            if (!stop_arrival && maxoff + 1 > 2 * nl_ - 1) continue;
            double cost = *std::max_element(load.begin(), load.end());
            if (cost < best) {
                best = cost;
                layer_off = loff;
                rt_off = roff;
                stop_off = stop_arrival ? -1 : maxoff + 1;
                lag_max = maxoff;
            }
        }
        return best < 1e300;
    };
    if (lag_ok && place(steps) && (stop_arrival ? lag_max >= steps : stop_off >= steps)) {
        nlaunch = steps;
        lagged = true;
    } else {
        nlaunch = steps + 1;
        stop_off = -1;
        layer_off.assign(n_targets, steps);
        rt_off.assign((size_t)(ri1 - ri0), steps);
    }
    std::vector<int64_t> uoffs(2 * nlaunch + 1, 0), roffs(2 * nlaunch + 1, 0);
    {
        std::vector<std::vector<CleUnit>> ub(2 * nlaunch);
        for (const CleUnit& u : units) ub[layer_off[chunks[u.chunk].layer]].push_back(u);
        units.clear();
        for (int32_t k = 0; k < 2 * nlaunch; ++k) {
            uoffs[k] = (int64_t)units.size();
            units.insert(units.end(), ub[k].begin(), ub[k].end());
        }
        uoffs[2 * nlaunch] = (int64_t)units.size();
        if (fused) {
            std::vector<std::vector<CleTask>> rb(2 * nlaunch);
            for (int64_t t = ri0; t < ri1; ++t) rb[rt_off[t - ri0]].push_back(rt[t]);
            rt.resize(ri0);
            for (int32_t k = 0; k < 2 * nlaunch; ++k) {
                roffs[k] = (int64_t)rt.size();
                rt.insert(rt.end(), rb[k].begin(), rb[k].end());
            }
            roffs[2 * nlaunch] = (int64_t)rt.size();
            ri1 = (int64_t)rt.size();
        }
    }
    S.R = std::move(R);
    S.M = M;
    S.chains = chains;
    S.steps = steps;
    S.fused = fused;
    S.rt = std::move(rt);
    S.at = std::move(at);
    S.rstep = std::move(rstep);
    S.astep = std::move(astep);
    S.ri0 = ri0;
    S.ri1 = ri1;
    S.layers = std::move(layers);
    S.chunks = std::move(chunks);
    S.units = std::move(units);
    S.b1off = std::move(b1off);
    S.nb1_total = nb1_total;
    S.uoffs = std::move(uoffs);
    S.roffs = std::move(roffs);
    S.nlaunch = nlaunch;
    S.stop_off = stop_off;
    S.lagged = lagged;
    S.id = ++g_struct_ids;
    for (const CleTask& tk : S.at) {
        const CleRel& q = S.R[tk.rel];
        const int64_t n = tk.b - tk.a;
        switch (tk.kind) {
            case kApplyW1: S.bytes_rescale += 8 * n * q.len1; break;
            case kApplyW2Contig:
            case kApplyDwBoth: S.bytes_rescale += 8 * n * q.o2g * q.khw2; break;
            case kApplyW2Tile: S.bytes_rescale += 8 * n * (tk.c1 - tk.c0) * q.khw2; break;
            default:
                S.bytes_rescale += 8 * n * ((q.b1 ? 1 : 0) + (q.bnw ? 1 : 0) + (q.bnb ? 1 : 0) + (q.sacc ? 1 : 0));
        }
    }
    for (int32_t l = 0; l < n_targets; ++l) S.bytes_metric += 12 * target_n[l];
    {
        const int64_t r0 = fused ? S.ri0 : 0, r1 = fused ? S.ri1 : (int64_t)S.rt.size();
        for (int64_t t = r0; t < r1; ++t) {
            const CleTask& tk = S.rt[t];
            const CleRel& q = S.R[tk.rel];
            const int64_t n = tk.b - tk.a;
            if (tk.kind == kRangeW1) S.bytes_range += 4 * n * q.len1;
            else if (tk.kind == kRangeW2Contig) S.bytes_range += 4 * n * q.o2g * q.khw2;
            else if (tk.kind == kRangeW2Tile) S.bytes_range += 4 * n * (tk.c1 - tk.c0) * q.khw2;
        }
    }
    const double tp5 = now_us();
    S.t_chains = tp2 - tp1;
    S.t_tasks = tp3 - tp2;
    S.t_chunks = tp4 - tp3;
    S.t_place = tp5 - tp4;
    return DFQ_OK;
}

static std::vector<int64_t> cle_structure_key(const std::vector<CleRel>& R, int64_t M, float* const* targets,
                                              const int64_t* target_n, int32_t n_targets, int32_t ref_threads) {
    std::vector<std::pair<uintptr_t, int32_t>> ps;
    ps.reserve(5 * R.size() + n_targets);
    for (const CleRel& c : R)
        for (const void* q : {(const void*)c.w1, (const void*)c.w2, (const void*)c.b1, (const void*)c.bnw,
                              (const void*)c.bnb})
            ps.push_back({reinterpret_cast<uintptr_t>(q), (int32_t)ps.size()});
    for (int32_t l = 0; l < n_targets; ++l) ps.push_back({reinterpret_cast<uintptr_t>(targets[l]), (int32_t)ps.size()});
    std::vector<int32_t> id(ps.size());
    std::vector<std::pair<uintptr_t, int32_t>> srt = ps;
    std::sort(srt.begin(), srt.end());
    for (size_t i = 0; i < srt.size();) {
        size_t j = i;
        while (j < srt.size() && srt[j].first == srt[i].first) ++j;
        for (size_t k = i; k < j; ++k) id[srt[k].second] = srt[i].first ? srt[i].second : -1;
        i = j;
    }
    std::vector<int64_t> key;
    key.reserve(16 * R.size() + 2 * n_targets + 16);
    key.push_back((int64_t)R.size());
    key.push_back(M);
    key.push_back(n_targets);
    key.push_back(ref_threads);
    for (const char* sw : {"DFQ_CLE_FUSED", "DFQ_CLE_LAG", "DFQ_CLE_BAND", "DFQ_CLE_STOP",
                           "DFQ_CLE_W1_ROWS", "DFQ_CLE_DW_ROWS"}) {
        const char* v = ab_env(sw);
        int64_t h = v ? 1 : 0;
        for (int k = 0; v && v[k] && k < 8; ++k) h = h * 131 + (unsigned char)v[k];
        key.push_back(h);
    }
    size_t q = 0;
    for (const CleRel& c : R) {
        key.insert(key.end(), {c.c1, c.len1, c.o2, c.i2, c.khw2, (int64_t)c.sacc_init, (int64_t)c.vec1, (int64_t)c.vec2,
                               (int64_t)(c.sacc != nullptr)});
        for (int k = 0; k < 5; ++k) key.push_back(id[q++]);
    }
    for (int32_t l = 0; l < n_targets; ++l) {
        key.push_back(target_n[l]);
        key.push_back(id[q++]);
    }
    return key;
}

static int cle_rels_from_desc(const dfq_cle_rel* rels, int32_t n_rel, std::vector<CleRel>& R, int64_t& M) {
    R.assign(n_rel, CleRel{});
    M = 0;
    for (int32_t r = 0; r < n_rel; ++r) {
        const dfq_cle_rel& d = rels[r];
        if (!d.w1 || !d.w2 || !d.b1 || d.c1 <= 0 || d.len1 <= 0 || d.o2 <= 0 || d.i2 <= 0 || d.khw2 <= 0)
            return DFQ_ERR_INVALID;
        int64_t groups = 1;
        if (d.c1 != d.i2) {
            groups = d.c1 / d.i2;
            if (groups <= 0 || groups * d.i2 != d.c1) return DFQ_ERR_SHAPE;
        }
        if (d.o2 % groups != 0) return DFQ_ERR_SHAPE;
        CleRel c{};
        c.w1 = d.w1; c.w2 = d.w2; c.b1 = d.b1; c.bnw = d.bn_w; c.bnb = d.bn_b; c.sacc = d.s_acc;
        c.c1 = d.c1; c.len1 = d.len1; c.o2 = d.o2; c.i2 = d.i2; c.khw2 = d.khw2; c.o2g = d.o2 / groups;
        c.moff = M;
        c.sacc_init = d.s_acc_init;
        c.vec1 = (d.len1 % 4 == 0 && reinterpret_cast<uintptr_t>(d.w1) % 16 == 0) ? 1 : 0;
        c.vec2 = (d.i2 == 1 && (c.o2g * d.khw2) % 4 == 0 && reinterpret_cast<uintptr_t>(d.w2) % 16 == 0) ? 1 : 0;
        c.fuse_next = -1;
        c.dw_prev = -1;
        c.w1_self = 0;
        c.w2_self = 0;
        M += 2 * d.c1;
        R[r] = c;
    }
    return DFQ_OK;
}

static std::mutex g_struct_mu;
static std::list<std::pair<std::vector<int64_t>, std::shared_ptr<const CleStructure>>> g_struct_cache;
constexpr size_t kStructCacheCap = 8;

extern "C" int dfq_cle_plan_create(const dfq_cle_rel* rels, int32_t n_rel, float* const* targets,
                                   const int64_t* target_n, int32_t n_targets, double s_min, double s_max,
                                   int32_t is_signed, float eps, int32_t ref_threads, void* ws, int64_t ws_bytes,
                                   dfq_cle_plan** out) {
    if (!out || n_rel < 0 || n_targets < 0 || (n_rel > 0 && !rels) || (n_targets > 0 && (!targets || !target_n)))
        return DFQ_ERR_INVALID;
    const double tc0 = now_us();
    const int64_t need_ws = dfq_cle_plan_ws_bytes(target_n, n_targets);
    if (need_ws < 0) return DFQ_ERR_INVALID;
    if (ws && (ws_bytes < need_ws || reinterpret_cast<uintptr_t>(ws) % 256 != 0)) return DFQ_ERR_INVALID;
    *out = nullptr;
    std::vector<CleRel> R;
    int64_t M = 0;
    if (const int rc = cle_rels_from_desc(rels, n_rel, R, M); rc != DFQ_OK) return rc;
    const double tp1 = now_us();
    std::shared_ptr<const CleStructure> S;
    bool cached = false;
    const std::vector<int64_t> key = cle_structure_key(R, M, targets, target_n, n_targets, ref_threads);
    {
        std::lock_guard<std::mutex> lock(g_struct_mu);
        for (auto it = g_struct_cache.begin(); it != g_struct_cache.end(); ++it)
            if (it->first == key) {
                S = it->second;
                g_struct_cache.splice(g_struct_cache.begin(), g_struct_cache, it);
                cached = true;
                break;
            }
    }
    if (!S) {
        auto built = std::make_shared<CleStructure>();
        const int rc = cle_build_structure(R, M, n_rel, targets, target_n, n_targets, ref_threads, *built);
        if (rc != DFQ_OK) return rc;
        S = built;
        std::lock_guard<std::mutex> lock(g_struct_mu);
        g_struct_cache.emplace_front(key, S);
        if (g_struct_cache.size() > kStructCacheCap) g_struct_cache.pop_back();
    }
    const double tp5 = now_us();
    std::vector<CleRel> Rb = S->R;
    for (int32_t r = 0; r < n_rel; ++r) {
        Rb[r].w1 = R[r].w1; Rb[r].w2 = R[r].w2; Rb[r].b1 = R[r].b1;
        Rb[r].bnw = R[r].bnw; Rb[r].bnb = R[r].bnb; Rb[r].sacc = R[r].sacc;
    }
    dfq_cle_plan* p = new (std::nothrow) dfq_cle_plan();
    if (!p) return DFQ_ERR_NOMEM;
    std::vector<CleLayer> layers = S->layers;
    {
        char* snap_base = static_cast<char*>(ws);
        if (!snap_base && need_ws > 0) {
            hipError_t e = hipMalloc(&p->d_snap_owned, need_ws);
            if (e != hipSuccess) { set_last_hip_error(e); cle_plan_free(p); return DFQ_ERR_HIP; }
            snap_base = static_cast<char*>(p->d_snap_owned);
        }
        int64_t snap_off = 0;
        for (int32_t l = 0; l < n_targets; ++l) {
            layers[l].w = targets[l];
            layers[l].snap = reinterpret_cast<float*>(snap_base + snap_off);
            snap_off += snap_bytes(target_n[l]);
        }
    }
    const std::vector<CleTask>& rt = S->rt;
    const std::vector<CleTask>& at = S->at;
    const std::vector<CleChunk>& chunks = S->chunks;
    const std::vector<CleUnit>& units = S->units;
    const std::vector<int64_t>& b1off = S->b1off;
    const std::vector<int64_t>& rstep = S->rstep;
    const std::vector<int64_t>& astep = S->astep;
    const int64_t nb1_total = S->nb1_total, ri0 = S->ri0, ri1 = S->ri1;
    const int32_t steps = S->steps, chains = S->chains, nlaunch = S->nlaunch, stop_off = S->stop_off;
    const bool fused = S->fused, lagged = S->lagged;
    if (cle_timing() && !cached) {
        fprintf(stderr, "DFQ_CLE_TIMING plan: steps %d nlaunch %d lagged %d stop %d; offsets (units/ranges):", steps,
                nlaunch, (int)lagged, stop_off);
        for (int32_t k = 0; k < 2 * nlaunch; ++k)
            fprintf(stderr, " %d:%lld/%lld", k, (long long)(S->uoffs[k + 1] - S->uoffs[k]),
                    (long long)(S->roffs[k + 1] - S->roffs[k]));
        fprintf(stderr, "; rescale tasks per step:");
        for (int32_t k = 0; k < steps; ++k) fprintf(stderr, " %lld", (long long)(astep[k + 1] - astep[k]));
        fprintf(stderr, "\n");
    }
    (void)hipGetDevice(&p->dev);
    p->uoffs = S->uoffs;
    p->roffs = S->roffs;
    p->nlaunch = nlaunch;
    p->lagged = lagged;
    p->stop_off = stop_off;
    p->nunits = (int64_t)units.size();
    p->M = M;
    p->nl = n_targets;
    p->nchunks = (int64_t)chunks.size();
    p->chains = chains;
    p->steps = steps;
    p->fused = fused;
    p->rstep = rstep;
    p->astep = astep;
    p->step_pos.assign(std::max<int32_t>(steps, 1), 0);
    for (int32_t k = 0; k < steps; ++k)
        for (int64_t t = astep[k]; t < astep[k + 1]; ++t)
            if (at[t].kind == kApplyW2Tile && Rb[at[t].rel].khw2 > 1) p->step_pos[k] = 1;
    p->ri0 = ri0;
    p->ri1 = ri1;
    p->bytes[0] = S->bytes_rescale;
    p->bytes[1] = S->bytes_metric;
    p->bytes[2] = S->bytes_range;
#ifdef DFQ_DIAGNOSTICS
    if (ab_env("DFQ_CLE_TL")) {
        p->h_rels = R;
        p->h_atasks = at;
    }
#endif
    p->smin = s_min; p->smax = s_max; p->is_signed = is_signed; p->eps = eps;
    hipError_t e;
    auto fail = [&](hipError_t err) { set_last_hip_error(err); cle_plan_free(p); return DFQ_ERR_HIP; };
    TableLayout T;
    const int64_t o_rels = T.add<CleRel>((int64_t)R.size());
    const int64_t o_rt = T.add<CleTask>((int64_t)rt.size());
    const int64_t o_at = T.add<CleTask>((int64_t)at.size());
    const int64_t o_layers = T.add<CleLayer>((int64_t)layers.size());
    const int64_t o_chunks = T.add<CleChunk>((int64_t)chunks.size());
    const int64_t o_units = T.add<CleUnit>((int64_t)units.size());
    const int64_t o_b1off = T.add<int64_t>((int64_t)b1off.size());
    p->slots = std::max<int32_t>(ref_threads, 1);
    const int64_t o_part = T.add<float>((int64_t)(p->slots + 2) * n_targets);
    const int64_t host_bytes = T.total;
    const int64_t o_b1 = T.add<float>(32 * nb1_total);
    const int64_t o_tail = T.add<float>(kCleTailWords * (int64_t)chunks.size());
    const int64_t o_rng = T.add<uint32_t>(4 * M);
    const int64_t o_means = T.add<double>(n_targets);
    const int64_t o_state = T.add<CleState>(1);
    const int64_t o_hist = T.add<double>(kCleHistCap);
    const int64_t o_cnt = T.add<uint32_t>((int64_t)chunks.size() + 1);
    const int64_t o_vsave = T.add<float>(lagged ? 2 * M : 0);
    const int64_t o_vtag = T.add<int32_t>(lagged ? (int64_t)at.size() : 0);
    const double tm0 = now_us();
    char* base = nullptr;
    char* hblob = nullptr;
    CleDeviceCtx& ctx = cle_device_ctx(p->dev);
    e = hipSuccess;
    {
        std::lock_guard<std::mutex> lock(ctx.mu);
        if (!ctx.pool_busy && (e = cle_ctx_ready(ctx)) == hipSuccess &&
            (e = hipEventSynchronize(ctx.pool_ev)) == hipSuccess) {
            if (ctx.pool_cap < (size_t)T.total) {
                (void)hipFree(ctx.d_pool);
                ctx.d_pool = nullptr;
                ctx.pool_cap = 0;
                ctx.pool_struct = 0;
                const size_t cap = (size_t)T.total + (size_t)T.total / 2;
                if ((e = hipMalloc(&ctx.d_pool, cap)) == hipSuccess) ctx.pool_cap = cap;
            }
            if (e == hipSuccess && ctx.hpool_cap < (size_t)host_bytes) {
                (void)hipHostFree(ctx.h_pool);
                ctx.h_pool = nullptr;
                ctx.hpool_cap = 0;
                const size_t cap = (size_t)host_bytes + (size_t)host_bytes / 2;
                if ((e = hipHostMalloc(&ctx.h_pool, cap, hipHostMallocDefault)) == hipSuccess) ctx.hpool_cap = cap;
            }
            if (e == hipSuccess) {
                ctx.pool_busy = true;
                p->pooled = true;
                base = ctx.d_pool;
                hblob = ctx.h_pool;
            }
        }
        if (e != hipSuccess) return fail(e);
    }
    std::vector<char> blob;
    const bool resident = p->pooled && ctx.pool_struct == S->id;
    if (!p->pooled) {
        if ((e = hipMalloc(&p->d_tables, T.total)) != hipSuccess) return fail(e);
        base = static_cast<char*>(p->d_tables);
        blob.assign(host_bytes, 0);
        hblob = blob.data();
    } else if (!resident) {
        std::memset(hblob, 0, host_bytes);
    }
    const double tm1 = now_us();
    auto put = [&](int64_t off, const auto& v) {
        if (!v.empty()) std::memcpy(hblob + off, v.data(), sizeof(v[0]) * v.size());
    };
    put(o_rels, Rb);
    put(o_layers, layers);
    if (!resident) {
        put(o_rt, rt); put(o_at, at); put(o_chunks, chunks); put(o_units, units); put(o_b1off, b1off);
        float* lm = reinterpret_cast<float*>(hblob + o_part) + (int64_t)p->slots * n_targets;
        for (int64_t l = 0; l < n_targets; ++l) {
            lm[2 * l] = (float)layers[l].n;
            lm[2 * l + 1] = layers[l].nt == 1 ? 1.f : 0.f;
        }
    }
    if (p->pooled) {
        if (resident) {
            const size_t nr = sizeof(CleRel) * Rb.size(), nly = sizeof(CleLayer) * layers.size();
            if (nr && (e = hipMemcpyAsync(base + o_rels, hblob + o_rels, nr, hipMemcpyHostToDevice, ctx.st)) != hipSuccess)
                return fail(e);
            if (nly && (e = hipMemcpyAsync(base + o_layers, hblob + o_layers, nly, hipMemcpyHostToDevice, ctx.st)) !=
                           hipSuccess)
                return fail(e);
        } else if ((e = hipMemcpyAsync(base, hblob, host_bytes, hipMemcpyHostToDevice, ctx.st)) != hipSuccess) {
            return fail(e);
        }
        if ((e = hipEventRecord(ctx.pool_ev, ctx.st)) != hipSuccess) return fail(e);
        ctx.pool_struct = S->id;
    } else if ((e = hipMemcpy(base, hblob, host_bytes, hipMemcpyHostToDevice)) != hipSuccess) {
        return fail(e);
    }
    if (cle_timing())
        fprintf(stderr, "DFQ_CLE_TIMING create: plan %.1f us (relations %.1f, structure %s %.1f: chains %.1f, tasks %.1f, "
                "chunks %.1f, placement %.1f), tables %lld B %.1f us, copy %lld B %.1f us\n", tm0 - tc0, tp1 - tc0,
                cached ? "cached" : "built", tp5 - tp1, S->t_chains, S->t_tasks, S->t_chunks, S->t_place,
                (long long)T.total, tm1 - tm0, (long long)host_bytes, now_us() - tm1);
    p->d_rels = reinterpret_cast<CleRel*>(base + o_rels);
    p->d_rtasks = reinterpret_cast<CleTask*>(base + o_rt);
    p->d_atasks = reinterpret_cast<CleTask*>(base + o_at);
    p->d_layers = reinterpret_cast<CleLayer*>(base + o_layers);
    p->d_chunks = reinterpret_cast<CleChunk*>(base + o_chunks);
    p->d_units = reinterpret_cast<CleUnit*>(base + o_units);
    p->d_b1off = reinterpret_cast<int64_t*>(base + o_b1off);
    p->d_b1 = reinterpret_cast<float*>(base + o_b1);
    p->d_tail = reinterpret_cast<float*>(base + o_tail);
    p->d_rng = reinterpret_cast<uint32_t*>(base + o_rng);
    p->d_part = reinterpret_cast<float*>(base + o_part);
    p->d_means = reinterpret_cast<double*>(base + o_means);
    p->d_state = reinterpret_cast<CleState*>(base + o_state);
    p->d_hist = p->d_hist_tables = reinterpret_cast<double*>(base + o_hist);
    p->d_cnt = reinterpret_cast<uint32_t*>(base + o_cnt);
    p->n_at = (int64_t)at.size();
    if (lagged) {
        p->d_vsave = reinterpret_cast<float*>(base + o_vsave);
        p->d_vtag = reinterpret_cast<int32_t*>(base + o_vtag);
    }
    for (const auto& c : chunks) p->nbig += c.len >= 8 ? 1 : 0;
    *out = p;
    return DFQ_OK;
}

static int cle_enqueue_iteration(dfq_cle_plan* p, hipStream_t s, int32_t g, int32_t max_iters) {
    const int64_t kStepGrid = [] {
        const char* e = ab_env("DFQ_CLE_STEP_GRID");
        return e && *e ? std::max<int64_t>(1, atoll(e)) : int64_t(2048);
    }();
    const int64_t kTileGrid = [] {
        const char* e = ab_env("DFQ_CLE_TILE_GRID");
        return e && *e ? std::max<int64_t>(1, atoll(e)) : int64_t(4096);
    }();
    CleFin F{p->d_cnt, p->d_part, p->d_means, p->d_hist, p->nchunks, p->nbig, p->slots, p->nl, 0, p->d_flag,
             p->stop_off < 0 ? 1 : 0};
    const int32_t NL = p->nlaunch;
    const bool run_g = g < max_iters, prev = g >= 1;
    for (int32_t k = 0; k < NL; ++k) {
        const bool step = k < p->steps;
        const int64_t a0 = step ? p->astep[k] : 0, a1 = step ? p->astep[k + 1] : 0;
        if (step && run_g && !p->fused && p->rstep[k + 1] > p->rstep[k]) {
            hipLaunchKernelGGL(cle_loop_range_kernel, dim3((int)std::min<int64_t>(p->rstep[k + 1] - p->rstep[k], kStepGrid)),
                               dim3(kThreads), 0, s, p->d_rels, p->d_rtasks, p->rstep[k], p->rstep[k + 1], p->d_rng,
                               p->M, p->d_state, 0);
            DFQ_LAUNCH_CHECK();
        }
        const int64_t nab = run_g ? std::min<int64_t>(a1 - a0, kStepGrid) : 0;
        const int64_t uo = p->uoffs[k], nuo = run_g ? p->uoffs[k + 1] - uo : 0;
        const int64_t up = p->uoffs[NL + k], nup = prev ? p->uoffs[NL + k + 1] - up : 0;
        const int64_t ro = p->roffs[k], nro_t = (g + 1 < max_iters) ? p->roffs[k + 1] - ro : 0;
        const int64_t rp = p->roffs[NL + k], nrp_t = (prev && run_g) ? p->roffs[NL + k + 1] - rp : 0;
        int64_t nto = std::min<int64_t>(nuo, kTileGrid);
        const int64_t ntp = std::min<int64_t>(nup, kTileGrid);
        F.last = (k == p->steps) ? 1 : 0;
        if (F.last && run_g && p->nbig == 0) nto = std::max<int64_t>(nto, 1);
        const int64_t nro = std::min<int64_t>(nro_t, kStepGrid), nrp = std::min<int64_t>(nrp_t, kStepGrid);
        int32_t stop_it = -1;
        if (p->stop_off == k && run_g) stop_it = g;
        else if (p->stop_off == NL + k && prev) stop_it = g - 1;
        const int64_t nblk = nab + (stop_it >= 0 ? cle_stop_blocks(p->nchunks) : 0) + nto + ntp + nro + nrp;
        if (nblk == 0) continue;
        auto kern = (step && p->step_pos[k]) ? cle_loop_step_kernel<true> : cle_loop_step_kernel<false>;
        hipLaunchKernelGGL(kern, dim3((int)nblk), dim3(kThreads), 0, s, p->d_rels, p->d_atasks, a0, a1, nab, p->d_rng,
                           p->M, p->is_signed, p->eps, p->smin, p->smax, p->d_layers, p->d_chunks, p->d_b1off,
                           p->d_units, uo, nuo, nto, up, nup, ntp, p->d_b1, p->d_tail, p->d_rtasks, ro, nro_t, nro, rp,
                           nrp_t, nrp, F, p->d_state, g, p->d_vsave, p->d_vtag, stop_it);
        DFQ_LAUNCH_CHECK();
    }
    return DFQ_OK;
}

constexpr int32_t kCleAhead = 1;
constexpr double kClePollQuietUs = 1000.0;
static constexpr int kCleGateSeconds = 120;
static constexpr int kCleJoinSeconds = kCleGateSeconds + 30;
static constexpr double kCleLaunchDeadlineUs = 0.5e6 * kCleGateSeconds;
static hipError_t cle_hist_ready(CleDeviceCtx& ctx, int32_t max_iters) {
    if (ctx.h_hist_cap < max_iters + 1) {
        (void)hipHostFree(ctx.h_hist);
        ctx.h_hist = nullptr;
        ctx.h_hist_cap = 0;
        const hipError_t e = hipHostMalloc(&ctx.h_hist, sizeof(double) * (max_iters + 1), hipHostMallocDefault);
        if (e != hipSuccess) return e;
        ctx.h_hist_cap = max_iters + 1;
    }
    if (max_iters + 1 <= kCleHistCap || ctx.hist_cap >= max_iters + 1) return hipSuccess;
    (void)hipFree(ctx.d_hist);
    ctx.d_hist = nullptr;
    ctx.hist_cap = 0;
    const hipError_t e = hipMalloc(&ctx.d_hist, sizeof(double) * (max_iters + 1));
    if (e == hipSuccess) ctx.hist_cap = max_iters + 1;
    return e;
}

static hipError_t cle_copy_back(void* dst, const void* src, size_t bytes, hipStream_t s) {
    hipError_t e = hipMemcpyAsync(dst, src, bytes, hipMemcpyDeviceToHost, s);
    return e == hipSuccess ? hipStreamSynchronize(s) : e;
}

static int cle_run_locked(dfq_cle_plan* p, CleDeviceCtx& ctx, double threshold, int32_t count, int32_t max_iters,
                          int32_t* iterations, std::vector<double>* hist, double deadline_us = -1.0) {
    DFQ_HIP_CHECK(cle_ctx_ready(ctx));
    p->st = ctx.st;
    p->h_state = ctx.h_state;
    *ctx.h_flag = 0;
    p->d_flag = ctx.d_flag;
    hipStream_t s = p->st;
    p->d_hist = p->d_hist_tables;
    DFQ_HIP_CHECK(cle_hist_ready(ctx, max_iters));
    if (max_iters + 1 > kCleHistCap) p->d_hist = ctx.d_hist;
    CleState init{};
    init.diff = 1e8;
    init.thr = threshold;
    init.iter_count = 0;
    init.iters = 0;
    init.count = count;
    init.max_iters = max_iters;
    init.done = !((init.diff > threshold) && (0 < count)) || max_iters == 0;
    {
        const int64_t npart = (int64_t)p->slots * std::max(p->nl, 1), ncnt = p->nchunks + 1;
        const int64_t nvtag = p->d_vtag ? p->n_at : 0;
        const int64_t words = std::max({4 * p->M, npart, ncnt, nvtag});
        const int64_t grid = std::min<int64_t>(std::max<int64_t>({p->nunits, ceil_div(words, (int64_t)kThreads), 1}), 4096);
        hipLaunchKernelGGL(cle_loop_init_kernel, dim3((int)grid), dim3(kThreads), 0, s, p->d_layers, p->d_chunks,
                           p->nchunks, p->d_units, p->nunits, p->d_rng, p->M, p->d_part, npart, p->d_cnt, ncnt,
                           p->d_vtag, nvtag, p->d_state, init);
        DFQ_LAUNCH_CHECK();
    }
    if (p->fused && p->rstep[1] > p->rstep[0]) {
        hipLaunchKernelGGL(cle_loop_range_kernel, dim3((int)std::min<int64_t>(p->rstep[1] - p->rstep[0], 2048)),
                           dim3(kThreads), 0, s, p->d_rels, p->d_rtasks, p->rstep[0], p->rstep[1], p->d_rng, p->M,
                           p->d_state, 0);
        DFQ_LAUNCH_CHECK();
    }
#ifdef DFQ_DIAGNOSTICS
    uint64_t* d_tl = nullptr;
    uint64_t* d_tl2 = nullptr;
    const int64_t n_at = p->astep.empty() ? 0 : p->astep.back();
    const size_t n_tl2 = 4 * (size_t)(kCleTl2Fin + 1);
    {
        const char* e = ab_env("DFQ_CLE_TILES_FIRST");
        const int tf = e && *e ? (e[0] == '1' ? 1 : 0) : (kCleTilesFirst ? 1 : 0);
        DFQ_HIP_CHECK(hipMemcpyToSymbolAsync(HIP_SYMBOL(g_cle_tiles_first), &tf, sizeof(tf), 0, hipMemcpyHostToDevice, s));
    }
    if (ab_env("DFQ_CLE_TL") && n_at > 0) {
        DFQ_HIP_CHECK(hipMalloc(&d_tl, sizeof(uint64_t) * 4 * n_at));
        DFQ_HIP_CHECK(hipMemsetAsync(d_tl, 0, sizeof(uint64_t) * 4 * n_at, s));
        DFQ_HIP_CHECK(hipMemcpyToSymbolAsync(HIP_SYMBOL(g_cle_tl), &d_tl, sizeof(d_tl), 0, hipMemcpyHostToDevice, s));
        DFQ_HIP_CHECK(hipMalloc(&d_tl2, sizeof(uint64_t) * n_tl2));
        DFQ_HIP_CHECK(hipMemsetAsync(d_tl2, 0, sizeof(uint64_t) * n_tl2, s));
        DFQ_HIP_CHECK(hipMemcpyToSymbolAsync(HIP_SYMBOL(g_cle_tl2), &d_tl2, sizeof(d_tl2), 0, hipMemcpyHostToDevice, s));
        const char* ek = ab_env("DFQ_CLE_TL_STEP");
        const int kk = ek && *ek ? atoi(ek) : -1;
        const int64_t a0v = (kk >= 0 && kk < p->steps) ? p->astep[kk] : -1;
        DFQ_HIP_CHECK(hipMemcpyToSymbolAsync(HIP_SYMBOL(g_cle_tl2_a0), &a0v, sizeof(a0v), 0, hipMemcpyHostToDevice, s));
        DFQ_HIP_CHECK(hipStreamSynchronize(s));
    }
#endif
    const double tc1 = now_us();
    int32_t launched = 0;
    bool deadline_hit = false;
    hipEvent_t tev[2] = {nullptr, nullptr};
    p->loop_ms = -1.f;
    if (p->timed) {
        DFQ_HIP_CHECK(hipEventCreate(&tev[0]));
        DFQ_HIP_CHECK(hipEventCreate(&tev[1]));
        DFQ_HIP_CHECK(hipEventRecord(tev[0], s));
    }
#ifdef DFQ_DIAGNOSTICS
    const char* pd = ab_env("DFQ_CLE_TEST_POLL_DELAY_US");
    const int poll_delay_us = pd ? atoi(pd) : 0;
    const double quiet_us = pd ? 0.0 : kClePollQuietUs;
#else
    const double quiet_us = kClePollQuietUs;
#endif
    if (!init.done) {
        uint32_t last_f = ~0u;
        double t_moved = tc1;
        for (;;) {
            const uint32_t f = __atomic_load_n(ctx.h_flag, __ATOMIC_ACQUIRE);
            if (f & 1u) break;
            const int32_t ran = (int32_t)(f >> 1);
            if (launched <= max_iters && !deadline_hit && launched - ran <= kCleAhead) {
                const int rc = cle_enqueue_iteration(p, s, launched, max_iters);
                if (rc != DFQ_OK) return rc;
                ++launched;
                continue;
            }
#ifdef DFQ_DIAGNOSTICS
            if (poll_delay_us > 0) std::this_thread::sleep_for(std::chrono::microseconds(poll_delay_us));
#endif
            const double t = now_us();
            if (f != last_f) {
                last_f = f;
                t_moved = t;
            } else if (t - t_moved >= quiet_us) {
                const hipError_t q = hipStreamQuery(s);
                if (q != hipErrorNotReady) {
                    if (q != hipSuccess) break;
                    const uint32_t f2 = __atomic_load_n(ctx.h_flag, __ATOMIC_ACQUIRE);
                    if ((f2 & 1u) || launched > max_iters || deadline_hit || (int32_t)(f2 >> 1) + 1 < launched) break;
                }
                t_moved = t;
            }
            if (deadline_us > 0 && t - tc1 > deadline_us) deadline_hit = true;
            __builtin_ia32_pause();
        }
    }
    if (!init.done && p->lagged) {
        hipLaunchKernelGGL(cle_loop_rollback_kernel, dim3(1024), dim3(kThreads), 0, s, p->d_layers, p->nl, p->d_rels,
                           p->d_atasks, p->n_at, p->d_vsave, p->d_vtag, p->d_state);
        DFQ_LAUNCH_CHECK();
    }
    if (tev[1]) DFQ_HIP_CHECK(hipEventRecord(tev[1], s));
    if (p->d_sig) DFQ_HIP_CHECK(hipStreamWriteValue64(s, p->d_sig, p->gen, 0));
    DFQ_HIP_CHECK(hipMemcpyAsync(p->h_state, p->d_state, sizeof(CleState), hipMemcpyDeviceToHost, s));
    const int32_t hn = std::min(launched, max_iters);
    if (hist && hn > 0) DFQ_HIP_CHECK(hipMemcpyAsync(ctx.h_hist, p->d_hist, sizeof(double) * hn, hipMemcpyDeviceToHost, s));
    DFQ_HIP_CHECK(hipStreamSynchronize(s));
    p->launched = launched;
    if (tev[0]) {
        float ms = -1.f;
        if (hipEventElapsedTime(&ms, tev[0], tev[1]) == hipSuccess) p->loop_ms = ms;
        (void)hipEventDestroy(tev[0]);
        (void)hipEventDestroy(tev[1]);
    }
    if (cle_timing())
        fprintf(stderr, "DFQ_CLE_TIMING run: loop %.1f us (%d iterations launched)\n", now_us() - tc1, launched);
#ifdef DFQ_DIAGNOSTICS
    if (d_tl) {
        std::vector<uint64_t> tl(4 * (size_t)n_at);
        DFQ_HIP_CHECK(cle_copy_back(tl.data(), d_tl, sizeof(uint64_t) * tl.size(), s));
        uint64_t* null_tl = nullptr;
        DFQ_HIP_CHECK(hipMemcpyToSymbolAsync(HIP_SYMBOL(g_cle_tl), &null_tl, sizeof(null_tl), 0, hipMemcpyHostToDevice, s));
        std::vector<uint64_t> tl2(n_tl2);
        DFQ_HIP_CHECK(cle_copy_back(tl2.data(), d_tl2, sizeof(uint64_t) * n_tl2, s));
        DFQ_HIP_CHECK(hipMemcpyToSymbolAsync(HIP_SYMBOL(g_cle_tl2), &null_tl, sizeof(null_tl), 0, hipMemcpyHostToDevice, s));
        DFQ_HIP_CHECK(hipStreamSynchronize(s));
        (void)hipFree(d_tl2);
        {
            uint64_t t0 = ~0ull;
            for (int b = 0; b < kCleTl2Fin; ++b)
                if (tl2[4 * b]) t0 = std::min(t0, tl2[4 * b]);
            fprintf(stderr, "DFQ_CLE_TL last launch%s:", ab_env("DFQ_CLE_TL_STEP") ? " of DFQ_CLE_TL_STEP" : "");
            for (int role = 1; role <= 3; ++role) {
                std::vector<double> st, en, du;
                for (int b = 0; b < kCleTl2Fin; ++b) {
                    const uint64_t* r = &tl2[4 * b];
                    if (!r[0] || (int)r[2] != role) continue;
                    st.push_back((double)(r[0] - t0) * 0.01);
                    en.push_back((double)(r[1] - t0) * 0.01);
                    du.push_back((double)(r[1] - r[0]) * 0.01);
                }
                if (st.empty()) continue;
                std::sort(st.begin(), st.end());
                std::sort(en.begin(), en.end());
                double m = 0;
                for (double x : du) m += x;
                fprintf(stderr, " [%s: %zu blocks, start p50 %.2f max %.2f, end p50 %.2f max %.2f, dur mean %.2f]",
                        role == 1 ? "tiles" : role == 2 ? "ranges" : "tail tiles", st.size(), st[st.size() / 2], st.back(), en[en.size() / 2],
                        en.back(), m / du.size());
            }
            const uint64_t* f = &tl2[4 * kCleTl2Fin];
            if (f[0] && t0 != ~0ull)
                fprintf(stderr, " [stop rule: %.2f - %.2f, sums staged %.2f, means %.2f]", (double)(f[0] - t0) * 0.01,
                        (double)(f[1] - t0) * 0.01, f[2] ? (double)(f[2] - t0) * 0.01 : -1.0,
                        f[3] ? (double)(f[3] - t0) * 0.01 : -1.0);
            fprintf(stderr, "\n");
        }
        DFQ_HIP_CHECK(hipStreamSynchronize(s));
        (void)hipFree(d_tl);
        for (int32_t k = 0; k < p->steps; ++k) {
            const int64_t a0 = p->astep[k], a1 = p->astep[k + 1];
            uint64_t t_lo = ~0ull, t_hi = 0;
            double sum = 0;
            std::vector<std::pair<double, int64_t>> d;
            for (int64_t t = a0; t < a1; ++t) {
                const uint64_t* r = &tl[4 * t];
                if (!r[0]) continue;
                t_lo = std::min(t_lo, r[0]);
                t_hi = std::max(t_hi, r[1]);
                const double us = (double)(r[1] - r[0]) * 0.01;
                sum += us;
                d.push_back({us, t});
            }
            std::sort(d.rbegin(), d.rend());
            fprintf(stderr, "DFQ_CLE_TL step %d: %lld tasks, span %.2f us, task mean %.2f us, max %.2f us; slowest:",
                    k, (long long)(a1 - a0), t_hi > t_lo ? (double)(t_hi - t_lo) * 0.01 : 0.0,
                    d.empty() ? 0.0 : sum / d.size(), d.empty() ? 0.0 : d[0].first);
            for (size_t i = 0; i < d.size() && i < 6; ++i) {
                const uint64_t m = tl[4 * d[i].second + 3];
                const int rel = (int)((m >> 8) & 0xffff);
                const CleRel& q = p->h_rels[rel];
                const CleTask& tk = p->h_atasks[d[i].second];
                fprintf(stderr, " [%.2f us kind %d rel %d n %lld c1 %lld o2 %lld i2 %lld khw2 %lld o2g %lld fuse %d cols %lld",
                        d[i].first, (int)(m & 255), rel, (long long)(m >> 24), (long long)q.c1, (long long)q.o2,
                        (long long)q.i2, (long long)q.khw2, (long long)q.o2g, q.fuse_next, (long long)(tk.c1 - tk.c0));
                const uint64_t sub = tl[4 * d[i].second + 2];
                if (sub >> 63)
                    fprintf(stderr, q.khw2 > 1 ? " scales %.2f inv_pos %.2f rows %.2f" : " landed %.2f rows %.2f barrier %.2f",
                            (double)(sub & 0xffff) * 0.01, (double)((sub >> 16) & 0xffff) * 0.01,
                            (double)((sub >> 32) & 0xffff) * 0.01);
                fprintf(stderr, "]");
            }
            fprintf(stderr, "\nDFQ_CLE_TL step %d starts (us after first):", k);
            std::vector<double> st;
            for (int64_t t = a0; t < a1; ++t)
                if (tl[4 * t]) st.push_back((double)(tl[4 * t] - t_lo) * 0.01);
            std::sort(st.begin(), st.end());
            for (double q : {0.1, 0.5, 0.9, 0.99, 1.0})
                if (!st.empty()) fprintf(stderr, " p%.0f %.2f", q * 100, st[std::min(st.size() - 1, (size_t)(q * st.size()))]);
            fprintf(stderr, "\nDFQ_CLE_TL step %d kinds:", k);
            for (int kind = 0; kind < 8; ++kind) {
                int64_t cnt = 0;
                double sum = 0, mx = 0, s0 = 0;
                for (int64_t t = a0; t < a1; ++t) {
                    const uint64_t* r = &tl[4 * t];
                    if (!r[0] || (int)(r[3] & 255) != kind) continue;
                    const double us = (double)(r[1] - r[0]) * 0.01;
                    ++cnt;
                    sum += us;
                    mx = std::max(mx, us);
                    s0 += (double)(r[0] - t_lo) * 0.01;
                }
                if (cnt)
                    fprintf(stderr, " [kind %d: %lld tasks, mean %.2f max %.2f us, start mean %.2f]", kind,
                            (long long)cnt, sum / cnt, mx, s0 / cnt);
            }
            fprintf(stderr, "\n");
        }
    }
#endif
    const CleState fin = *p->h_state;
    if (fin.error) {
        set_last_hip_error(hipErrorLaunchTimeOut);
        return DFQ_ERR_HIP;
    }
    if (!fin.done) {
        set_last_hip_error_text(deadline_hit ? "the launched CLE loop reached its time limit before converging"
                                             : "the CLE loop stopped before its stop rule said done");
        return DFQ_ERR_HIP;
    }
    if (ab_env("DFQ_CLE_DEBUG")) {
        std::vector<float> part((size_t)p->slots * std::max(p->nl, 1));
        DFQ_HIP_CHECK(cle_copy_back(part.data(), p->d_part, sizeof(float) * part.size(), s));
        for (int32_t l = 0; l < p->nl; ++l) {
            fprintf(stderr, "DFQ_CLE_DEBUG layer %d:", l);
            for (int t = 0; t < p->slots; ++t) fprintf(stderr, " %.9g", part[(size_t)p->slots * l + t]);
            fprintf(stderr, "\n");
        }
    }
    if (iterations) *iterations = fin.iters;
    if (hist) {
        hist->assign((size_t)std::max(fin.iters, 0), 0.0);
        if (fin.iters > 0) std::memcpy(hist->data(), ctx.h_hist, sizeof(double) * std::min(fin.iters, hn));
    }
    return DFQ_OK;
}

extern "C" int dfq_cle_plan_run(dfq_cle_plan* p, double threshold, int32_t count, int32_t max_iters,
                                int32_t* iterations, double* diffs, void* stream) {
    if (!p || max_iters < 0 || p->async) return DFQ_ERR_INVALID;
    const double ts0 = now_us();
    DFQ_HIP_CHECK(hipStreamSynchronize(static_cast<hipStream_t>(stream)));
    const double ts1 = now_us();
    int dev = 0;
    DFQ_HIP_CHECK(hipGetDevice(&dev));
    CleDeviceCtx& ctx = cle_device_ctx(dev);
    std::lock_guard<std::mutex> lock(ctx.mu);
    if (cle_timing()) fprintf(stderr, "DFQ_CLE_TIMING run: caller sync %.1f us, context %.1f us\n", ts1 - ts0,
                              now_us() - ts1);
    std::vector<double> h;
    const int rc = cle_run_locked(p, ctx, threshold, count, max_iters, iterations, diffs ? &h : nullptr);
    if (rc == DFQ_OK && diffs && !h.empty()) std::memcpy(diffs, h.data(), sizeof(double) * h.size());
    return rc;
}

namespace dfq {
__global__ void __launch_bounds__(64) cle_caller_gate_kernel(const uint64_t* sig, uint64_t gen, uint64_t limit) {
    if (threadIdx.x != 0) return;
    const uint64_t t0 = __builtin_amdgcn_s_memrealtime();
    while (__hip_atomic_load(sig, __ATOMIC_RELAXED, __HIP_MEMORY_SCOPE_SYSTEM) < gen) {
        if (__builtin_amdgcn_s_memrealtime() - t0 > limit) __builtin_trap();
        __builtin_amdgcn_s_sleep(32);
    }
    __atomic_thread_fence(__ATOMIC_ACQUIRE);
}
}


struct CleAsync {
    std::mutex m;
    std::condition_variable cv;
    bool done = false;
    int rc = DFQ_OK;
    int32_t iters = 0;
    std::vector<double> hist;
    char err[128] = {0};
};

struct CleWorker {
    std::mutex m;
    std::condition_variable cv;
    std::function<void()> job;
    bool has_job = false;
};
static void cle_worker_loop(CleWorker* w) {
    for (;;) {
        std::function<void()> j;
        {
            std::unique_lock<std::mutex> l(w->m);
            w->cv.wait(l, [w] { return w->has_job; });
            j = std::move(w->job);
            w->has_job = false;
        }
        j();
    }
}

static hipError_t cle_signal_ready(CleDeviceCtx& ctx) {
    if (ctx.sig) return hipSuccess;
    if (ctx.sig_state < 0) return hipErrorNotSupported;
    hipError_t e = hipSuccess;
    void* sig = nullptr;
    if ((e = hipExtMallocWithFlags(&sig, sizeof(uint64_t), hipMallocSignalMemory)) != hipSuccess) {
        ctx.sig_state = -1;
        return e;
    }
    if ((e = hipStreamWriteValue64(ctx.st, sig, 0, 0)) != hipSuccess || (e = hipStreamSynchronize(ctx.st)) != hipSuccess) {
        (void)hipFree(sig);
        ctx.sig_state = -1;
        return e;
    }
    ctx.sig = sig;
    ctx.gen = 0;
    return hipSuccess;
}

static bool cle_async_join(dfq_cle_plan* p, double seconds = -1.0) {
    if (!p || !p->async) return true;
    CleAsync* a = p->async;
    std::unique_lock<std::mutex> l(a->m);
    if (seconds < 0) {
        a->cv.wait(l, [a] { return a->done; });
        return true;
    }
    return a->cv.wait_for(l, std::chrono::duration<double>(seconds), [a] { return a->done; });
}

extern "C" int dfq_cle_plan_launch(dfq_cle_plan* p, double threshold, int32_t count, int32_t max_iters,
                                   void* stream) {
    if (!p || max_iters < 0 || p->async) return DFQ_ERR_INVALID;
    if (ab_env("DFQ_CLE_TL")) return DFQ_ERR_UNSUPPORTED;
    hipStream_t caller = static_cast<hipStream_t>(stream);
    CleDeviceCtx& ctx = cle_device_ctx(p->dev);
    const double tl0 = now_us();
    if (ctx.pending && ctx.pending != p) cle_async_join(ctx.pending);
    ctx.pending = nullptr;
    uint64_t gen = 0;
    {
        std::lock_guard<std::mutex> lock(ctx.mu);
        DFQ_HIP_CHECK(hipSetDevice(p->dev));
        DFQ_HIP_CHECK(cle_ctx_ready(ctx));
        const hipError_t es = cle_signal_ready(ctx);
        if (es == hipErrorNotSupported) return DFQ_ERR_UNSUPPORTED;
        DFQ_HIP_CHECK(es);
        DFQ_HIP_CHECK(cle_hist_ready(ctx, max_iters));
        DFQ_HIP_CHECK(hipEventRecord(ctx.in_ev, caller));
        DFQ_HIP_CHECK(hipStreamWaitEvent(ctx.st, ctx.in_ev, 0));
        gen = ctx.gen + 1;
        hipLaunchKernelGGL(cle_caller_gate_kernel, dim3(1), dim3(64), 0, caller,
                           static_cast<const uint64_t*>(ctx.sig), gen, (uint64_t)kCleGateSeconds * 100000000ull);
        DFQ_LAUNCH_CHECK();
        ctx.gen = gen;
    }
    if (cle_timing()) fprintf(stderr, "DFQ_CLE_TIMING launch: gate and order %.1f us\n", now_us() - tl0);
    CleAsync* a = new (std::nothrow) CleAsync();
    const double t_launch = now_us();
    auto body = [p, &ctx, threshold, count, max_iters, gen, t_launch](CleAsync* a) {
        std::lock_guard<std::mutex> lock(ctx.mu);
        int rc = DFQ_OK;
        if (hipSetDevice(p->dev) != hipSuccess) {
            rc = DFQ_ERR_HIP;
        } else {
            rc = cle_run_locked(p, ctx, threshold, count, max_iters, &a->iters, &a->hist, kCleLaunchDeadlineUs);
        }
        if (rc == DFQ_ERR_HIP) {
            const char* m = dfq_last_hip_error();
            for (size_t i = 0; m && m[i] && i + 1 < sizeof(a->err); ++i) a->err[i] = m[i];
        }
#ifdef DFQ_DIAGNOSTICS
        if (const char* d = ab_env("DFQ_CLE_TEST_RELEASE_DELAY_MS"))
            std::this_thread::sleep_for(std::chrono::milliseconds(atoi(d)));
#endif
        hipError_t e = hipStreamWriteValue64(ctx.st, ctx.sig, gen, 0);
        if (e == hipSuccess) e = hipStreamSynchronize(ctx.st);
        if (e != hipSuccess) {
            fprintf(stderr, "dfq_cle_plan_launch: releasing the caller's stream failed (%s)\n", hipGetErrorString(e));
            if (rc == DFQ_OK) rc = DFQ_ERR_HIP;
        }
        if (rc == DFQ_OK && now_us() - t_launch > 0.9e6 * kCleGateSeconds) {
            set_last_hip_error(hipErrorLaunchTimeOut);
            const char* m = "CLE loop outlived the caller's stream gate";
            for (size_t i = 0; m[i] && i + 1 < sizeof(a->err); ++i) a->err[i] = m[i];
            rc = DFQ_ERR_HIP;
        }
        {
            std::lock_guard<std::mutex> l(a->m);
            a->rc = rc;
            a->done = true;
        }
        a->cv.notify_all();
    };
    if (!a) {
        CleAsync tmp;
        body(&tmp);
        return tmp.rc;
    }
    p->async = a;
    ctx.pending = p;
    p->d_sig = static_cast<uint64_t*>(ctx.sig);
    if (ab_env("DFQ_CLE_HOST_RELEASE")) p->d_sig = nullptr;
    p->gen = gen;
    bool posted = false;
    try {
        if (!ctx.worker) {
            CleWorker* w = new CleWorker();
            std::thread(cle_worker_loop, w).detach();
            ctx.worker = w;
        }
        {
            std::lock_guard<std::mutex> l(ctx.worker->m);
            ctx.worker->job = [body, a] { body(a); };
            ctx.worker->has_job = true;
        }
        ctx.worker->cv.notify_one();
        posted = true;
    } catch (...) {
    }
    if (!posted) body(a);
    if (cle_timing()) fprintf(stderr, "DFQ_CLE_TIMING launch: total %.1f us\n", now_us() - tl0);
    return DFQ_OK;
}

extern "C" int dfq_cle_plan_join(dfq_cle_plan* p, int32_t* iterations, double* diffs) {
    if (!p || !p->async) return DFQ_ERR_INVALID;
    if (p->abandoned) return DFQ_ERR_HIP;
    double limit = kCleJoinSeconds;
#ifdef DFQ_DIAGNOSTICS
    if (const char* j = ab_env("DFQ_CLE_TEST_JOIN_LIMIT_MS")) limit = atoi(j) * 1e-3;
#endif
    if (!cle_async_join(p, limit)) {
        p->abandoned = true;
        set_last_hip_error_text("the launched CLE loop did not finish in time; the caller's stream stays held");
        return DFQ_ERR_HIP;
    }
    CleDeviceCtx& ctx = cle_device_ctx(p->dev);
    if (ctx.pending == p) ctx.pending = nullptr;
    const CleAsync& a = *p->async;
    if (a.rc == DFQ_ERR_HIP && a.err[0]) set_last_hip_error_text(a.err);
    if (a.rc != DFQ_OK) return a.rc;
    if (iterations) *iterations = a.iters;
    if (diffs && !a.hist.empty()) std::memcpy(diffs, a.hist.data(), sizeof(double) * a.hist.size());
    return DFQ_OK;
}

extern "C" int dfq_cle_plan_info(const dfq_cle_plan* p, int32_t* chains, int32_t* steps, int32_t* launches) {
    if (!p) return DFQ_ERR_INVALID;
    if (chains) *chains = p->chains;
    if (steps) *steps = p->steps;
    if (launches) *launches = p->fused ? p->nlaunch : 2 * p->steps + 1;
    return DFQ_OK;
}

extern "C" int dfq_cle_plan_set_timing(dfq_cle_plan* p, int32_t on) {
    if (!p || p->async) return DFQ_ERR_INVALID;
    p->timed = on != 0;
    return DFQ_OK;
}

extern "C" int dfq_cle_plan_stats(const dfq_cle_plan* p, int64_t* bytes, double* loop_ms, int32_t* launched) {
    if (!p) return DFQ_ERR_INVALID;
    if (bytes) {
        bytes[0] = p->bytes[0];
        bytes[1] = p->bytes[1];
        bytes[2] = p->bytes[2];
    }
    if (loop_ms) *loop_ms = p->loop_ms;
    if (launched) *launched = p->launched;
    return DFQ_OK;
}

extern "C" int dfq_cle_plan_destroy(dfq_cle_plan* p) {
    if (!p) return DFQ_OK;
    if (p->abandoned) return DFQ_OK;
    if (p->async) {
        cle_async_join(p);
        CleDeviceCtx& ctx = cle_device_ctx(p->dev);
        if (ctx.pending == p) ctx.pending = nullptr;
        delete p->async;
        p->async = nullptr;
    }
    cle_plan_free(p);
    return DFQ_OK;
}


namespace dfq {
constexpr size_t kClePreloadPool = size_t(4) << 20, kClePreloadHostPool = size_t(2) << 20;
constexpr int32_t kClePreloadHistIters = 100000;
hipError_t preload_cle() {
    int dev = 0;
    hipError_t e0 = hipGetDevice(&dev);
    if (e0 != hipSuccess) return e0;
    {
        CleDeviceCtx& ctx = cle_device_ctx(dev);
        std::lock_guard<std::mutex> lock(ctx.mu);
        if ((e0 = cle_ctx_ready(ctx)) != hipSuccess) return e0;
        if (!ctx.pool_busy && ctx.pool_cap < kClePreloadPool) {
            (void)hipFree(ctx.d_pool);
            ctx.d_pool = nullptr;
            ctx.pool_cap = 0;
            ctx.pool_struct = 0;
            if ((e0 = hipMalloc(&ctx.d_pool, kClePreloadPool)) != hipSuccess) return e0;
            ctx.pool_cap = kClePreloadPool;
        }
        if (!ctx.pool_busy && ctx.hpool_cap < kClePreloadHostPool) {
            (void)hipHostFree(ctx.h_pool);
            ctx.h_pool = nullptr;
            ctx.hpool_cap = 0;
            if ((e0 = hipHostMalloc(&ctx.h_pool, kClePreloadHostPool, hipHostMallocDefault)) != hipSuccess) return e0;
            ctx.hpool_cap = kClePreloadHostPool;
        }
        if ((e0 = cle_hist_ready(ctx, kClePreloadHistIters)) != hipSuccess) return e0;
        (void)cle_signal_ready(ctx);
        if (!ctx.worker) {
            try {
                CleWorker* w = new CleWorker();
                std::thread(cle_worker_loop, w).detach();
                ctx.worker = w;
            } catch (...) {
            }
        }
    }
    hipFuncAttributes a;
    hipError_t e = hipFuncGetAttributes(&a, reinterpret_cast<const void*>(cle_loop_step_kernel<true>));
    if (e == hipSuccess) e = hipFuncGetAttributes(&a, reinterpret_cast<const void*>(cle_loop_step_kernel<false>));
    return e;
}
}

#ifdef DFQ_DIAGNOSTICS
#include "dfq_diag.h"
extern "C" int dfq_diag_cle_check_structure(const dfq_cle_rel* rels, int32_t n_rel, float* const* targets,
                                            const int64_t* target_n, int32_t n_targets, int32_t ref_threads,
                                            int64_t* info, char* msg, int32_t msg_cap) {
    auto fail = [&](const char* fmt, long long a, long long b, long long c) {
        if (msg && msg_cap > 0) snprintf(msg, (size_t)msg_cap, fmt, a, b, c);
        return DFQ_ERR_INVALID;
    };
    if (n_rel < 0 || n_targets < 0 || (n_rel > 0 && !rels) || (n_targets > 0 && (!targets || !target_n)))
        return fail("bad arguments %lld %lld %lld", n_rel, n_targets, 0);
    std::vector<CleRel> R0;
    int64_t M = 0;
    if (const int rc = cle_rels_from_desc(rels, n_rel, R0, M); rc != DFQ_OK) return rc;
    CleStructure S;
    if (const int rc = cle_build_structure(R0, M, n_rel, targets, target_n, n_targets, ref_threads, S); rc != DFQ_OK)
        return rc;
    const std::vector<CleRel>& R = S.R;
    const int32_t steps = S.steps, NL = S.nlaunch;
    if (const char* e = getenv("DFQ_CLE_PLACE_DUMP"); e && *e) {
        fprintf(stderr, "DFQ_CLE_PLACE steps %d nlaunch %d lagged %d stop_off %d\n", steps, NL, (int)S.lagged,
                S.stop_off);
        for (int32_t k = 0; k < 2 * NL; ++k) {
            int64_t na = 0;
            double ba = 0;
            if (k < steps)
                for (int64_t t = S.astep[k]; t < S.astep[k + 1]; ++t, ++na) {
                    const CleTask& tk = S.at[t];
                    const CleRel& q = R[tk.rel];
                    const int64_t n = tk.b - tk.a;
                    if (tk.kind == kApplyW1) ba += 8.0 * n * q.len1;
                    else if (tk.kind == kApplyW2Tile) ba += 8.0 * n * (tk.c1 - tk.c0) * q.khw2;
                    else if (tk.kind != kApplyChannels) ba += 8.0 * n * q.o2g * q.khw2;
                }
            double bu = 0;
            for (int64_t u = S.uoffs[k]; u < S.uoffs[k + 1]; ++u) {
                const CleChunk& ch = S.chunks[S.units[u].chunk];
                const int64_t nb1 = ch.len / kCleTile;
                bu += 12.0 * (S.units[u].tile < nb1 ? kCleTile : ch.len - nb1 * kCleTile);
            }
            double br = 0;
            for (int64_t t = S.roffs[k]; t < S.roffs[k + 1]; ++t) {
                const CleTask& tk = S.rt[t];
                const CleRel& q = R[tk.rel];
                const int64_t n = tk.b - tk.a;
                if (tk.kind == kRangeW1) br += 4.0 * n * q.len1;
                else if (tk.kind == kRangeW2Contig) br += 4.0 * n * q.o2g * q.khw2;
                else if (tk.kind == kRangeW2Tile) br += 4.0 * n * (tk.c1 - tk.c0) * q.khw2;
            }
            fprintf(stderr, "DFQ_CLE_PLACE offset %d: rescale %lld blocks %.2f MB, tiles %lld blocks %.2f MB, ranges %lld blocks %.2f MB\n",
                    k, (long long)na, ba / 1e6, (long long)(S.uoffs[k + 1] - S.uoffs[k]), bu / 1e6,
                    (long long)(S.roffs[k + 1] - S.roffs[k]), br / 1e6);
        }
    }
    if (info) {
        const int64_t v[8] = {steps, NL, S.lagged ? 1 : 0, S.stop_off, (int64_t)S.at.size(), (int64_t)S.rt.size(),
                              (int64_t)S.units.size(), (int64_t)S.chunks.size()};
        std::memcpy(info, v, sizeof(v));
    }
    for (int32_t r = 0; r < n_rel; ++r) {
        const CleRel& c = R[r];
        if (c.moff < 0 || c.moff + 2 * c.c1 > S.M) return fail("rel %lld: range words [%lld, +2 c1) past M %lld", r, c.moff, S.M);
        if (2 * c.moff + 4 * c.c1 > 2 * S.M) return fail("rel %lld: rollback saves past 2 M (moff %lld, c1 %lld)", r, c.moff, c.c1);
        if (c.fuse_next >= n_rel || c.dw_prev >= n_rel || c.fuse_next < -1 || c.dw_prev < -1)
            return fail("rel %lld: link out of range (fuse_next %lld, dw_prev %lld)", r, c.fuse_next, c.dw_prev);
        if (c.fuse_next >= 0 && R[c.fuse_next].moff + R[c.fuse_next].c1 > S.M)
            return fail("rel %lld: fused W1 words of rel %lld past M %lld", r, c.fuse_next, S.M);
    }
    if ((int32_t)S.astep.size() != steps + 1 || S.astep[0] != 0 || S.astep.back() != (int64_t)S.at.size())
        return fail("astep: %lld entries for %lld steps, last %lld", (long long)S.astep.size(), steps,
                    S.astep.empty() ? -1 : S.astep.back());
    std::vector<int32_t> rel_step(n_rel, -1);
    std::vector<std::pair<const float*, int32_t>> touch;
    for (int32_t k = 0; k < steps; ++k) {
        if (S.astep[k + 1] < S.astep[k]) return fail("astep not monotone at step %lld: %lld > %lld", k, S.astep[k], S.astep[k + 1]);
        for (int64_t t = S.astep[k]; t < S.astep[k + 1]; ++t) {
            const CleTask& tk = S.at[t];
            if (tk.rel < 0 || tk.rel >= n_rel) return fail("rescale task %lld: relation %lld of %lld", t, tk.rel, n_rel);
            const CleRel& c = R[tk.rel];
            if (tk.a < 0 || tk.a >= tk.b) return fail("rescale task %lld: empty or negative span [%lld, %lld)", t, tk.a, tk.b);
            switch (tk.kind) {
                case kApplyW1:
                    if (tk.b > c.c1) return fail("W1 task %lld: rows to %lld of %lld", t, tk.b, c.c1);
                    touch.push_back({c.w1, k});
                    break;
                case kApplyW2Contig:
                    if (tk.b > c.c1 || c.i2 != 1) return fail("W2 contig task %lld: channels to %lld of %lld", t, tk.b, c.c1);
                    touch.push_back({c.w2, k});
                    break;
                case kApplyDwBoth:
                    if (tk.b > c.c1 || tk.c0 < 0 || tk.c0 >= n_rel || R[tk.c0].w1 != c.w2 || R[tk.c0].dw_prev != tk.rel)
                        return fail("depthwise pair task %lld: partner %lld, channels to %lld", t, tk.c0, tk.b);
                    touch.push_back({c.w2, k});
                    break;
                case kApplyW2Tile:
                    if (tk.b > c.o2 || tk.c0 < 0 || tk.c0 >= tk.c1 || tk.c1 > c.i2)
                        return fail("W2 tile task %lld: rows to %lld, columns to %lld", t, tk.b, tk.c1);
                    touch.push_back({c.w2, k});
                    break;
                case kApplyChannels:
                    if (tk.b > c.c1) return fail("channel task %lld: channels to %lld of %lld", t, tk.b, c.c1);
                    if (rel_step[tk.rel] >= 0 && rel_step[tk.rel] != k)
                        return fail("relation %lld: channel tasks in steps %lld and %lld", tk.rel, rel_step[tk.rel], k);
                    rel_step[tk.rel] = k;
                    break;
                default:
                    return fail("rescale task %lld: kind %lld", t, tk.kind, 0);
            }
        }
    }
    for (int32_t r = 0; r < n_rel; ++r)
        if (rel_step[r] < 0) return fail("relation %lld has no channel task", r, 0, 0);
    const int64_t nrt = (int64_t)S.rt.size();
    if (S.ri0 < 0 || S.ri0 > S.ri1 || S.ri1 > nrt) return fail("range slice [%lld, %lld) of %lld tasks", S.ri0, S.ri1, nrt);
    for (int64_t t = 0; t < nrt; ++t) {
        const CleTask& tk = S.rt[t];
        if (tk.rel < 0 || tk.rel >= n_rel) return fail("range task %lld: relation %lld of %lld", t, tk.rel, n_rel);
        const CleRel& c = R[tk.rel];
        if (tk.a < 0 || tk.a >= tk.b) return fail("range task %lld: span [%lld, %lld)", t, tk.a, tk.b);
        const bool ok = tk.kind == kRangeW2Tile ? (tk.b <= c.o2 && tk.c0 >= 0 && tk.c0 < tk.c1 && tk.c1 <= c.i2)
                                                : (tk.kind >= kRangeW1 && tk.kind <= kRangeResetW1 && tk.b <= c.c1);
        if (!ok) return fail("range task %lld (kind %lld): span to %lld out of the relation's shape", t, tk.kind, tk.b);
    }
    int64_t nb1_seen = 0;
    for (size_t ci = 0; ci < S.chunks.size(); ++ci) {
        const CleChunk& ch = S.chunks[ci];
        if (ch.layer < 0 || ch.layer >= n_targets) return fail("chunk %lld: layer %lld of %lld", (long long)ci, ch.layer, n_targets);
        if (ch.c0 < 0 || ch.len <= 0 || ch.c0 + ch.len > target_n[ch.layer])
            return fail("chunk %lld: elements [%lld, +%lld) past its layer", (long long)ci, ch.c0, ch.len);
        const int64_t nb1 = ch.len / 32 / 256;
        if (S.b1off[ci] != 32 * nb1_seen) return fail("chunk %lld: level-1 offset %lld, expected %lld", (long long)ci, S.b1off[ci], 32 * nb1_seen);
        nb1_seen += nb1;
    }
    if (nb1_seen != S.nb1_total) return fail("level-1 slots %lld, table %lld", nb1_seen, S.nb1_total, 0);
    for (size_t u = 0; u < S.units.size(); ++u) {
        const CleUnit& un = S.units[u];
        if (un.chunk < 0 || un.chunk >= (int32_t)S.chunks.size()) return fail("unit %lld: chunk %lld", (long long)u, un.chunk, 0);
        const CleChunk& ch = S.chunks[un.chunk];
        if (ch.len < 8 || un.tile < 0 || un.tile > ch.len / 32 / 256)
            return fail("unit %lld: tile %lld of chunk %lld", (long long)u, un.tile, un.chunk);
        const int64_t nb1 = ch.len / 32 / 256, e0 = (int64_t)un.tile * kCleTile;
        if (un.tile < nb1 ? e0 + kCleTile > ch.len : (ch.len - e0 < 0 || ch.len - e0 > kCleTile + kCleTailWords))
            return fail("unit %lld: tile past chunk %lld (len %lld)", (long long)u, un.chunk, ch.len);
    }
    if ((int32_t)S.uoffs.size() != 2 * NL + 1 || S.uoffs[0] != 0 || S.uoffs.back() != (int64_t)S.units.size())
        return fail("uoffs: %lld entries for %lld launches, last %lld", (long long)S.uoffs.size(), NL, S.uoffs.back());
    for (int32_t k = 0; k < 2 * NL; ++k)
        if (S.uoffs[k + 1] < S.uoffs[k]) return fail("uoffs not monotone at %lld", k, 0, 0);
    if (S.fused) {
        if ((int32_t)S.roffs.size() != 2 * NL + 1 || S.roffs[0] != S.ri0 || S.roffs.back() != S.ri1)
            return fail("roffs: %lld entries, [%lld, %lld)", (long long)S.roffs.size(), S.roffs.empty() ? -1 : S.roffs[0],
                        S.roffs.empty() ? -1 : S.roffs.back());
        for (int32_t k = 0; k < 2 * NL; ++k)
            if (S.roffs[k + 1] < S.roffs[k]) return fail("roffs not monotone at %lld", k, 0, 0);
    } else if ((int32_t)S.rstep.size() != steps + 1 || S.rstep.back() != nrt) {
        return fail("unfused rstep: %lld entries, last %lld of %lld", (long long)S.rstep.size(), S.rstep.back(), nrt);
    }
    if (NL != (S.lagged ? steps : steps + 1)) return fail("nlaunch %lld for %lld steps (lagged %lld)", NL, steps, S.lagged);
    auto span = [&](const float* w, int32_t& first, int32_t& last) {
        first = INT32_MAX;
        last = -1;
        for (const auto& x : touch)
            if (x.first == w) {
                first = std::min(first, x.second);
                last = std::max(last, x.second);
            }
        return last >= 0;
    };
    auto in_window = [&](const float* w, int32_t o) {
        int32_t f, l;
        if (!span(w, f, l)) return o >= 0 && o <= 2 * NL - 1;
        return o >= l + 1 && o <= std::min(2 * NL - 1, NL + f - 1);
    };
    int32_t umin = INT32_MAX, umax = -1;
    for (int32_t k = 0; k < 2 * NL; ++k)
        for (int64_t u = S.uoffs[k]; u < S.uoffs[k + 1]; ++u) {
            const int32_t l = S.chunks[S.units[u].chunk].layer;
            if (!S.lagged && k != steps) return fail("unit %lld of layer %lld at offset %lld outside the tiles-only launch", u, l, k);
            if (!in_window(targets[l], k)) return fail("unit %lld of layer %lld at offset %lld outside its tensor's window", u, l, k);
            umin = std::min(umin, k);
            umax = std::max(umax, k);
        }
    if (S.fused)
        for (int32_t k = 0; k < 2 * NL; ++k)
            for (int64_t t = S.roffs[k]; t < S.roffs[k + 1]; ++t) {
                const CleTask& tk = S.rt[t];
                const CleRel& c = R[tk.rel];
                bool ok = true;
                switch (tk.kind) {
                    case kRangeW1: ok = in_window(c.w1, k); break;
                    case kRangeW2Contig:
                    case kRangeW2Tile: ok = in_window(c.w2, k); break;
                    case kRangeReset: {
                        int32_t f, l;
                        span(c.w2, f, l);
                        ok = k >= rel_step[tk.rel] + 1 && k <= std::min(2 * NL - 1, NL + l);
                        break;
                    }
                    default: ok = k >= rel_step[tk.rel] + 1 && k <= 2 * NL - 1;
                }
                if (!S.lagged && k != steps) ok = false;
                if (!ok) return fail("range task %lld (kind %lld) at offset %lld outside its window", t, tk.kind, k);
            }
    if (S.lagged && S.stop_off >= 0) {
        if (S.stop_off < steps || S.stop_off > 2 * NL - 1) return fail("stop rule at offset %lld of [%lld, %lld]", S.stop_off, steps, 2 * NL - 1);
        if (umax >= 0 && S.stop_off <= umax) return fail("stop rule at offset %lld, not after the last tile offset %lld", S.stop_off, umax, 0);
        if (umax >= 0 && umin + NL <= S.stop_off)
            return fail("the next iteration's first tile (offset %lld + %lld) not after the stop rule at %lld", umin, NL, S.stop_off);
    } else if (!S.lagged && S.stop_off != -1) {
        return fail("unlagged plan with a stop-rule offset %lld", S.stop_off, 0, 0);
    }
    return DFQ_OK;
}
#endif
```

Measured before the change: 1944.

## Restructure CLE apply tile paths, tail-pass LDS staging, and kernel control flow

Turns the conditional loads in the range and scale helpers into predicated selects. Regroups the apply-tile branches so the single-group khw2==1 case is handled once, with an optional fused min/max. Makes the LDS struct templated so the position buffer can be dropped, and splits chunk-tail staging into multiple fixed-size passes with validation. Also joins any pending async plan before a synchronous run and reshapes the kernel's finish flow into a single exit point. These changes aim to cut divergence, LDS footprint and register pressure, at the cost of extra complexity and risk in the tail-pass index arithmetic.

```diff
diff --git a/data_free_quantization_amd/csrc/dfq_cle.hip b/data_free_quantization_amd/csrc/dfq_cle.hip
--- a/data_free_quantization_amd/csrc/dfq_cle.hip
+++ b/data_free_quantization_amd/csrc/dfq_cle.hip
@@ -95,8 +95,8 @@
     return v;
 }
 template <class F>
-__device__ __forceinline__ void for_short_rows(int64_t a, int64_t b, int64_t len, F&& f) {
-    const int lane = threadIdx.x & 63, wv = threadIdx.x >> 6;
+__device__ __forceinline__ void for_short_rows(int tid, int64_t a, int64_t b, int64_t len, F&& f) {
+    const int lane = tid & 63, wv = tid >> 6;
     const int G = row_group_lanes(len), rpw = 64 / G;
     const int sub = lane / G, sl = lane % G;
     for (int64_t base = a + (int64_t)wv * rpw; base < b; base += (int64_t)(kThreads / 64) * rpw) {
@@ -119,7 +119,7 @@
             f32x4 v[4];
 #pragma unroll
             for (int u = 0; u < 4; ++u)
-                if (i + 64 * u < n4) v[u] = p4[i + 64 * u];
+                v[u] = (i + 64 * u < n4) ? p4[i + 64 * u] : f32x4{0.f, 0.f, 0.f, 0.f};
 #pragma unroll
             for (int u = 0; u < 4; ++u)
                 if (i + 64 * u < n4) {
@@ -132,7 +132,7 @@
             float v[4];
 #pragma unroll
             for (int u = 0; u < 4; ++u)
-                if (i + 64 * u < n) v[u] = p[i + 64 * u];
+                v[u] = (i + 64 * u < n) ? p[i + 64 * u] : 0.f;
 #pragma unroll
             for (int u = 0; u < 4; ++u)
                 if (i + 64 * u < n) {
@@ -156,7 +156,7 @@
             f32x4 v[4];
 #pragma unroll
             for (int u = 0; u < 4; ++u)
-                if (i + 64 * u < n4) v[u] = p4[i + 64 * u];
+                v[u] = (i + 64 * u < n4) ? p4[i + 64 * u] : f32x4{0.f, 0.f, 0.f, 0.f};
             if (!have) {
                 f = factor();
                 have = true;
@@ -176,7 +176,7 @@
             float v[4];
 #pragma unroll
             for (int u = 0; u < 4; ++u)
-                if (i + 64 * u < n) v[u] = p[i + 64 * u];
+                v[u] = (i + 64 * u < n) ? p[i + 64 * u] : 0.f;
             if (!have) {
                 f = factor();
                 have = true;
@@ -203,7 +203,7 @@
             f32x4 v[4];
 #pragma unroll
             for (int u = 0; u < 4; ++u)
-                if (i + 64 * u < n4) v[u] = p4[i + 64 * u];
+                v[u] = (i + 64 * u < n4) ? p4[i + 64 * u] : f32x4{0.f, 0.f, 0.f, 0.f};
             if (!have) {
                 f = factor();
                 have = true;
@@ -225,7 +225,7 @@
             float v[4];
 #pragma unroll
             for (int u = 0; u < 4; ++u)
-                if (i + 64 * u < n) v[u] = p[i + 64 * u];
+                v[u] = (i + 64 * u < n) ? p[i + 64 * u] : 0.f;
             if (!have) {
                 f = factor();
                 have = true;
@@ -337,7 +337,7 @@
         uint32_t* mn = mins + R.moff;
         uint32_t* mx = maxs + R.moff;
         if (tk.kind == kRangeW1 && R.len1 < 64) {
-            for_short_rows(tk.a, tk.b, R.len1, [&](int64_t c, bool act, int sl, int G) {
+            for_short_rows(threadIdx.x, tk.a, tk.b, R.len1, [&](int64_t c, bool act, int sl, int G) {
                 float vmin = INFINITY, vmax = -INFINITY;
                 if (act)
                     for (int64_t i = sl; i < R.len1; i += G) {
@@ -354,7 +354,7 @@
             });
         } else if (tk.kind == kRangeW2Contig && R.o2g * R.khw2 < 64) {
             const int64_t seg = R.o2g * R.khw2;
-            for_short_rows(tk.a, tk.b, seg, [&](int64_t c, bool act, int sl, int G) {
+            for_short_rows(threadIdx.x, tk.a, tk.b, seg, [&](int64_t c, bool act, int sl, int G) {
                 float vmin = INFINITY, vmax = -INFINITY;
                 if (act)
                     for (int64_t i = sl; i < seg; i += G) {
@@ -401,7 +401,7 @@
                     float v[kColTileRows];
 #pragma unroll
                     for (int j = 0; j < kColTileRows; ++j)
-                        if (tk.a + j < tk.b) v[j] = ((DFQ_GLOBAL float*)R.w2)[(tk.a + j) * rowlen + i];
+                        v[j] = (tk.a + j < tk.b) ? ((DFQ_GLOBAL float*)R.w2)[(tk.a + j) * rowlen + i] : 0.f;
 #pragma unroll
                     for (int j = 0; j < kColTileRows; ++j)
                         if (tk.a + j < tk.b) {
@@ -464,10 +464,11 @@
                           smin, smax);
 }
 
+template <bool POS = true>
 struct CleApplyLds {
     float red[2][kThreads / 64][kColTileRows];
     float inv_s[kThreads];
-    float inv_pos[kThreads * kTileMaxKhw];
+    float inv_pos[POS ? kThreads * kTileMaxKhw : 1];
     float rows[kColTileRows * kThreads];
 };
 
@@ -482,7 +483,7 @@
 __device__ __forceinline__ void cle_apply_body(const CleRel* __restrict__ rels, const CleTask* __restrict__ tasks,
                                                int64_t t0, int64_t t1, uint32_t* __restrict__ rng, int64_t M,
                                                int par, bool first_iter, int is_signed, float eps, double smin,
-                                               double smax, int64_t blk, int64_t nblk, CleApplyLds& A,
+                                               double smax, int64_t blk, int64_t nblk, CleApplyLds<POS>& A,
                                                float* __restrict__ vsave = nullptr, int32_t* __restrict__ vtag = nullptr,
                                                int32_t iter = 0) {
     auto& red = A.red;
@@ -493,9 +494,11 @@
     uint32_t* maxs = mins + M;
     uint32_t* nmins = rng + (int64_t)(par ^ 1) * 2 * M;
     uint32_t* nmaxs = nmins + M;
-    const int lane = threadIdx.x & 63;
-    const int wv = threadIdx.x >> 6;
     for (int64_t t = t0 + blk; t < t1; t += nblk) {
+        int tid = threadIdx.x;
+        asm volatile("" : "+v"(tid));
+        const int lane = tid & 63;
+        const int wv = tid >> 6;
 #ifdef DFQ_DIAGNOSTICS
         const bool tl_on = g_cle_tl != nullptr;
         const uint64_t tl_start = tl_on ? __builtin_amdgcn_s_memrealtime() : 0;
@@ -510,7 +513,7 @@
         const uint32_t* mn = mins + R.moff;
         const uint32_t* mx = maxs + R.moff;
         if (tk.kind == kApplyW1 && R.len1 < 64) {
-            for_short_rows(tk.a, tk.b, R.len1, [&](int64_t c, bool act, int sl, int G) {
+            for_short_rows(tid, tk.a, tk.b, R.len1, [&](int64_t c, bool act, int sl, int G) {
                 float y0 = INFINITY, y1 = -INFINITY;
                 if (act && sl < R.len1) {
                     DFQ_GLOBAL float* p = (DFQ_GLOBAL float*)(R.w1 + c * R.len1 + sl);
@@ -531,7 +534,7 @@
         } else if (tk.kind == kApplyDwBoth && R.o2g * R.khw2 < 64) {
             const CleRel& N = rels[tk.c0];
             const int64_t seg = R.o2g * R.khw2;
-            for_short_rows(tk.a, tk.b, seg, [&](int64_t c, bool act, int sl, int G) {
+            for_short_rows(tid, tk.a, tk.b, seg, [&](int64_t c, bool act, int sl, int G) {
                 float z0 = INFINITY, z1 = -INFINITY;
                 if (act && sl < seg) {
                     DFQ_GLOBAL float* p = (DFQ_GLOBAL float*)(R.w2 + c * seg + sl);
@@ -555,7 +558,7 @@
         } else if (tk.kind == kApplyW2Contig && R.o2g * R.khw2 < 64) {
             const int64_t seg = R.o2g * R.khw2;
             const bool fuse = R.fuse_next >= 0;
-            for_short_rows(tk.a, tk.b, seg, [&](int64_t c, bool act, int sl, int G) {
+            for_short_rows(tid, tk.a, tk.b, seg, [&](int64_t c, bool act, int sl, int G) {
                 float vmin = INFINITY, vmax = -INFINITY;
                 if (act && sl < seg) {
                     DFQ_GLOBAL float* p = (DFQ_GLOBAL float*)(R.w2 + c * seg + sl);
@@ -628,7 +631,7 @@
                 }
             }
         } else if (POS && tk.kind == kApplyW2Tile && tile_by_position(R, tk) && tk.b - tk.a <= kPosTileMaxRows) {
-            const int t = threadIdx.x;
+            const int t = tid;
             const int khw = (int)R.khw2;
             const int64_t rowlen = R.i2 * R.khw2;
             const int ncol = (int)(tk.c1 - tk.c0);
@@ -684,36 +687,40 @@
                 atomicMax(&maxs[off], enc_ord(b));
             }
             __syncthreads();
-        } else if (tk.kind == kApplyW2Tile && R.fuse_next >= 0) {
-            const int64_t rowlen = R.i2 * R.khw2;
-            const int64_t i = tk.c0 + threadIdx.x;
-            const bool act = i < tk.c1;
-            const bool one_group = (tk.a / R.o2g) == ((tk.b - 1) / R.o2g);
+        } else if (tk.kind == kApplyW2Tile && (tk.a / R.o2g) == ((tk.b - 1) / R.o2g) && R.khw2 == 1) {
+            const bool fuse = R.fuse_next >= 0;
+            const int64_t rowlen = R.i2;
             const int nr = (int)(tk.b - tk.a);
-            if (one_group && R.khw2 == 1) {
+            DFQ_GLOBAL float* cb = (DFQ_GLOBAL float*)R.w2 + tk.a * rowlen + tk.c0;
+            const int64_t ncol = fuse ? (tk.c1 - tk.c0 < kThreads ? tk.c1 - tk.c0 : (int64_t)kThreads) : tk.c1 - tk.c0;
+            for (int64_t i0 = 0; i0 < ncol; i0 += kThreads) {
+                const uint32_t ti = (uint32_t)i0 + tid;
+                const bool act = ti < ncol;
                 float v[kColTileRows];
 #pragma unroll
-                for (int j = 0; j < kColTileRows; ++j)
-                    if (act && j < nr) v[j] = ((DFQ_GLOBAL float*)R.w2)[(tk.a + j) * rowlen + i];
+                for (int j = 0; j < kColTileRows; ++j) v[j] = (act && j < nr) ? (cb + j * rowlen)[ti] : 0.f;
                 const float inv =
-                    act ? cle_rel_scale(rels, R, mins, maxs, (tk.a / R.o2g) * R.i2 + i, is_signed, eps, smin, smax).inv : 0.f;
+                    act ? cle_rel_scale(rels, R, mins, maxs, (tk.a / R.o2g) * R.i2 + tk.c0 + ti, is_signed, eps, smin, smax).inv
+                        : 0.f;
 #pragma unroll
                 for (int j = 0; j < kColTileRows; ++j) {
                     if (j < nr) {
                         float y = __builtin_nanf("");
                         if (act) {
                             y = v[j] * inv;
-                            ((DFQ_GLOBAL float*)R.w2)[(tk.a + j) * rowlen + i] = y;
+                            (cb + j * rowlen)[ti] = y;
                         }
-                        rows[j * kThreads + threadIdx.x] = y;
+                        if (fuse) rows[j * kThreads + tid] = y;
                     }
                     if (j == 0) {
                         DFQ_CLE_TL_MARK(0)
                     }
                 }
                 DFQ_CLE_TL_MARK(1)
+            }
+            if (fuse) {
                 block_lds_sync();
-                const int r = threadIdx.x >> 4, sg = threadIdx.x & 15;
+                const int r = tid >> 4, sg = tid & 15;
                 float lo = INFINITY, hi = -INFINITY;
                 if (r < nr) {
                     const float4* q = reinterpret_cast<const float4*>(rows + r * kThreads + sg * 16);
@@ -738,66 +745,55 @@
                     atomicMin(&mins[off], enc_ord(lo));
                     atomicMax(&maxs[off], enc_ord(hi));
                 }
-            } else {
-                int64_t g_prev = -1;
-                float inv = 0.f;
-                for (int j = 0; j < nr; ++j) {
-                    const int64_t o = tk.a + j;
-                    float lo = INFINITY, hi = -INFINITY;
-                    if (act) {
-                        const int64_t g = o / R.o2g;
-                        if (g != g_prev) {
-                            inv = cle_rel_scale(rels, R, mins, maxs, g * R.i2 + i, is_signed, eps, smin, smax).inv;
-                            g_prev = g;
-                        }
-                        DFQ_GLOBAL float* p = (DFQ_GLOBAL float*)(R.w2 + o * rowlen + i * R.khw2);
-                        for (int64_t k = 0; k < R.khw2; ++k) {
-                            const float y = p[k] * inv;
-                            p[k] = y;
-                            lo = fminf(lo, y);
-                            hi = fmaxf(hi, y);
-                        }
+                __syncthreads();
+            }
+        } else if (tk.kind == kApplyW2Tile && R.fuse_next >= 0) {
+            const int64_t rowlen = R.i2 * R.khw2;
+            const int64_t i = tk.c0 + tid;
+            const bool act = i < tk.c1;
+            const int nr = (int)(tk.b - tk.a);
+            int64_t g_prev = -1;
+            float inv = 0.f;
+            for (int j = 0; j < nr; ++j) {
+                const int64_t o = tk.a + j;
+                float lo = INFINITY, hi = -INFINITY;
+                if (act) {
+                    const int64_t g = o / R.o2g;
+                    if (g != g_prev) {
+                        inv = cle_rel_scale(rels, R, mins, maxs, g * R.i2 + i, is_signed, eps, smin, smax).inv;
+                        g_prev = g;
                     }
-                    float a = lo, b = hi;
-                    cle_wave_minmax(a, b);
-                    if (lane == 0) {
-                        red[0][wv][j] = a;
-                        red[1][wv][j] = b;
+                    DFQ_GLOBAL float* p = (DFQ_GLOBAL float*)(R.w2 + o * rowlen + i * R.khw2);
+                    for (int64_t k = 0; k < R.khw2; ++k) {
+                        const float y = p[k] * inv;
+                        p[k] = y;
+                        lo = fminf(lo, y);
+                        hi = fmaxf(hi, y);
                     }
                 }
-                __syncthreads();
-                if (threadIdx.x < tk.b - tk.a) {
-                    const int j = threadIdx.x;
-                    float a = red[0][0][j], b = red[1][0][j];
-                    for (int w = 1; w < kThreads / 64; ++w) {
-                        a = fminf(a, red[0][w][j]);
-                        b = fmaxf(b, red[1][w][j]);
-                    }
-                    const int64_t off = rels[R.fuse_next].moff + tk.a + j;
-                    atomicMin(&mins[off], enc_ord(a));
-                    atomicMax(&maxs[off], enc_ord(b));
-                }
+                float a = lo, b = hi;
+                cle_wave_minmax(a, b);
+                if (lane == 0) {
+                    red[0][wv][j] = a;
+                    red[1][wv][j] = b;
+                }
+            }
+            __syncthreads();
+            if (tid < tk.b - tk.a) {
+                const int j = tid;
+                float a = red[0][0][j], b = red[1][0][j];
+                for (int w = 1; w < kThreads / 64; ++w) {
+                    a = fminf(a, red[0][w][j]);
+                    b = fmaxf(b, red[1][w][j]);
+                }
+                const int64_t off = rels[R.fuse_next].moff + tk.a + j;
+                atomicMin(&mins[off], enc_ord(a));
+                atomicMax(&maxs[off], enc_ord(b));
             }
             __syncthreads();
         } else if (tk.kind == kApplyW2Tile) {
             const int64_t rowlen = R.i2 * R.khw2;
-            const bool one_group = (tk.a / R.o2g) == ((tk.b - 1) / R.o2g);
-            for (int64_t i = tk.c0 + threadIdx.x; i < tk.c1; i += kThreads) {
-                if (one_group && R.khw2 == 1) {
-                    float v[kColTileRows];
-#pragma unroll
-                    for (int j = 0; j < kColTileRows; ++j)
-                        if (tk.a + j < tk.b) v[j] = ((DFQ_GLOBAL float*)R.w2)[(tk.a + j) * rowlen + i];
-                    const float inv = cle_rel_scale(rels, R, mins, maxs, (tk.a / R.o2g) * R.i2 + i, is_signed, eps, smin,
-                                                smax).inv;
-                    ((DFQ_GLOBAL float*)R.w2)[tk.a * rowlen + i] = v[0] * inv;
-                    DFQ_CLE_TL_MARK(0)
-#pragma unroll
-                    for (int j = 1; j < kColTileRows; ++j)
-                        if (tk.a + j < tk.b) ((DFQ_GLOBAL float*)R.w2)[(tk.a + j) * rowlen + i] = v[j] * inv;
-                    DFQ_CLE_TL_MARK(1)
-                    continue;
-                }
+            for (int64_t i = tk.c0 + tid; i < tk.c1; i += kThreads) {
                 int64_t g_prev = -1;
                 float inv = 0.f;
                 for (int64_t o = tk.a; o < tk.b; ++o) {
@@ -811,8 +807,8 @@
                 }
             }
         } else {
-            if (vtag && threadIdx.x == 0) vtag[t] = iter;
-            for (int64_t c = tk.a + threadIdx.x; c < tk.b; c += kThreads) {
+            if (vtag && tid == 0) vtag[t] = iter;
+            for (int64_t c = tk.a + tid; c < tk.b; c += kThreads) {
                 const CleScale cs = cle_rel_scale(rels, R, mins, maxs, c, is_signed, eps, smin, smax);
                 if (vsave) {
                     float* v = vsave + 2 * R.moff;
@@ -830,7 +826,7 @@
 #ifdef DFQ_DIAGNOSTICS
         if (tl_on) {
             __syncthreads();
-            if (threadIdx.x == 0) {
+            if (tid == 0) {
                 uint32_t hw, xcc;
                 asm volatile("s_getreg_b32 %0, hwreg(HW_REG_HW_ID)" : "=s"(hw));
                 asm volatile("s_getreg_b32 %0, hwreg(HW_REG_XCC_ID)" : "=s"(xcc));
@@ -847,6 +843,16 @@
 
 constexpr int kCleTile = 8192;
 constexpr int kCleTailWords = 64;
+constexpr int kCleL0Block = 512;
+constexpr int kCleTailPass = 4096;
+constexpr int kCleTailArea = 4096;
+static_assert(kCleTailPass % kCleL0Block == 0 && kCleTailPass <= kCleTailArea, "a tail pass: whole level-0 blocks inside the area");
+
+__host__ __device__ inline int64_t cle_tail_passes(int64_t rem_b0) { return rem_b0 / (kCleTailPass / kCleL0Block) + 1; }
+__host__ __device__ inline int64_t cle_tail_pass_count(int64_t cnt, int64_t pass) {
+    const int64_t left = cnt - pass * kCleTailPass;
+    return left < kCleTailPass ? left : kCleTailPass;
+}
 
 struct CleUnit {
     int32_t chunk;
@@ -905,26 +911,21 @@
         const int64_t e0 = (int64_t)un.tile * kCleTile;
         const int64_t cnt = full ? kCleTile : len - e0;
         if (full) {
-            float xs[2][16], ys[2][16];
-#pragma unroll
+#pragma unroll 1
             for (int h = 0; h < 2; ++h) {
                 const int q = tid + h * kThreads;
                 const int64_t base = e0 + 32 * (16 * (q >> 5)) + (q & 31);
+                float xs[16], ys[16];
 #pragma unroll
                 for (int j = 0; j < 16; ++j) {
-                    xs[h][j] = w[base + 32 * j];
-                    ys[h][j] = sn[base + 32 * j];
-                }
-            }
-#pragma unroll
-            for (int h = 0; h < 2; ++h) {
-                const int q = tid + h * kThreads;
-                const int64_t base = e0 + 32 * (16 * (q >> 5)) + (q & 31);
+                    xs[j] = w[base + 32 * j];
+                    ys[j] = sn[base + 32 * j];
+                }
                 float a = 0.f;
 #pragma unroll
                 for (int j = 0; j < 16; ++j) {
-                    a += fabsf(xs[h][j] - ys[h][j]);
-                    sn[base + 32 * j] = xs[h][j];
+                    a += fabsf(xs[j] - ys[j]);
+                    sn[base + 32 * j] = xs[j];
                 }
                 b0[q] = a;
             }
@@ -936,42 +937,55 @@
                 st_coh(b1buf + b1off[un.chunk] + (int64_t)un.tile * 32 + tid, a);
             }
         } else {
-            for (int64_t e = tid; e < cnt; e += 8 * kThreads) {
-                float x[8], y[8];
-#pragma unroll
-                for (int u = 0; u < 8; ++u)
-                    if (e + u * kThreads < cnt) {
-                        x[u] = w[e0 + e + u * kThreads];
-                        y[u] = sn[e0 + e + u * kThreads];
-                    }
-#pragma unroll
-                for (int u = 0; u < 8; ++u)
-                    if (e + u * kThreads < cnt) {
-                        d[e + u * kThreads] = fabsf(x[u] - y[u]);
-                        sn[e0 + e + u * kThreads] = x[u];
-                    }
-            }
-            __syncthreads();
             const int64_t ni = sz - nb1 * 256;
             const int64_t rem_b0 = ni / 16, tail0 = ni % 16;
             float* tb = tailbuf + (int64_t)un.chunk * kCleTailWords;
-            if (tid < 32) {
-                float a1p = 0.f;
-                for (int64_t m = 0; m < rem_b0; ++m) {
-                    float a = 0.f;
-                    for (int j = 0; j < 16; ++j) a += d[32 * (16 * m + j) + tid];
-                    a1p += a;
-                }
-                float a0t = 0.f;
-                for (int64_t j = 0; j < tail0; ++j) a0t += d[32 * (16 * rem_b0 + j) + tid];
-                float p = a0t;
-                p += a1p;
-                st_coh(tb + tid, p);
-            } else if (tid < 64) {
-                const int t = tid - 32;
-                const int64_t nv = vs - 4 * sz;
-                if (t < 24 && t < nv * 8) st_coh(tb + 32 + t, d[8 * (4 * sz) + t - e0]);
-                if (t < 8 && t < len - 8 * vs) st_coh(tb + 56 + t, d[8 * vs + t - e0]);
+            const int64_t npass = cle_tail_passes(rem_b0);
+            float a1p = 0.f;
+            for (int64_t ps = 0; ps < npass; ++ps) {
+                if (ps) __syncthreads();
+                const int64_t p0 = e0 + ps * kCleTailPass;
+                const int64_t pc = cle_tail_pass_count(cnt, ps);
+                for (int64_t e = tid; e < pc; e += 8 * kThreads) {
+                    float x[8], y[8];
+#pragma unroll
+                    for (int u = 0; u < 8; ++u)
+                    {
+                        const bool in = e + u * kThreads < pc;
+                        x[u] = in ? w[p0 + e + u * kThreads] : 0.f;
+                        y[u] = in ? sn[p0 + e + u * kThreads] : 0.f;
+                    }
+#pragma unroll
+                    for (int u = 0; u < 8; ++u)
+                        if (e + u * kThreads < pc) {
+                            d[e + u * kThreads] = fabsf(x[u] - y[u]);
+                            sn[p0 + e + u * kThreads] = x[u];
+                        }
+                }
+                __syncthreads();
+                const bool last = ps == npass - 1;
+                if (tid < 32) {
+                    constexpr int kPassBlocks = kCleTailPass / kCleL0Block;
+                    const int64_t mleft = rem_b0 - ps * kPassBlocks;
+                    const int64_t mp = mleft < kPassBlocks ? mleft : kPassBlocks;
+                    for (int64_t m = 0; m < mp; ++m) {
+                        float a = 0.f;
+                        for (int j = 0; j < 16; ++j) a += d[32 * (16 * m + j) + tid];
+                        a1p += a;
+                    }
+                    if (last) {
+                        float a0t = 0.f;
+                        for (int64_t j = 0; j < tail0; ++j) a0t += d[32 * (16 * mp + j) + tid];
+                        float p = a0t;
+                        p += a1p;
+                        st_coh(tb + tid, p);
+                    }
+                } else if (tid < 64 && last) {
+                    const int t = tid - 32;
+                    const int64_t nv = vs - 4 * sz;
+                    if (t < 24 && t < nv * 8) st_coh(tb + 32 + t, d[8 * (4 * sz) + t - p0]);
+                    if (t < 8 && t < len - 8 * vs) st_coh(tb + 56 + t, d[8 * vs + t - p0]);
+                }
             }
         }
         __syncthreads();
@@ -979,7 +993,7 @@
     }
 }
 
-constexpr int kCleTilesLds = kCleTile + kCleTailWords + 512;
+constexpr int kCleTilesLds = kCleTailArea + kCleTailWords + 512;
 constexpr int kCleRangeLds = 2 * kThreads * kTileMaxKhw;
 
 template <class LdB1, class LdTb>
@@ -1184,9 +1198,12 @@
     int32_t stop_arrival;
 };
 
-static_assert(kCleTilesLds - kCleTile >= kNpStackFloats, "np_pairwise's frame stack after the tile area");
+constexpr int kCleFinPart = 2048;
+constexpr int kCleFinStack = kCleTilesLds - kNpStackFloats;
+static_assert(kCleFinStack >= kCleFinPart && kCleFinStack % 2 == 0, "np_pairwise's frame stack behind the layer means, 8-B aligned");
+template <bool POS>
 union CleStepLds {
-    CleApplyLds apply;
+    CleApplyLds<POS> apply;
     float tiles[kCleTilesLds > kCleRangeLds ? kCleTilesLds : kCleRangeLds];
 };
 
@@ -1199,7 +1216,14 @@
 #ifndef DFQ_CLE_POS_WAVES
 #define DFQ_CLE_POS_WAVES 1
 #endif
-__global__ void __launch_bounds__(kThreads) __attribute__((amdgpu_waves_per_eu(POS ? DFQ_CLE_POS_WAVES : 4)))
+#ifndef DFQ_CLE_STEP_WAVES
+#define DFQ_CLE_STEP_WAVES 4
+#endif
+#ifndef DFQ_CLE_STEP_WAVES_MAX
+#define DFQ_CLE_STEP_WAVES_MAX 4
+#endif
+__global__ void __launch_bounds__(kThreads)
+    __attribute__((amdgpu_waves_per_eu(POS ? DFQ_CLE_POS_WAVES : DFQ_CLE_STEP_WAVES, POS ? 8 : DFQ_CLE_STEP_WAVES_MAX)))
 cle_loop_step_kernel(const CleRel* __restrict__ rels, const CleTask* __restrict__ atasks, int64_t a0, int64_t a1,
                      int64_t nab, uint32_t* __restrict__ rng, int64_t M, int is_signed, float eps, double smin,
                      double smax, const CleLayer* __restrict__ layers, const CleChunk* __restrict__ chunks,
@@ -1208,7 +1232,7 @@
                      float* __restrict__ tailbuf, const CleTask* __restrict__ rtasks, int64_t ro, int64_t nro_t,
                      int64_t nro, int64_t rp, int64_t nrp_t, int64_t nrp, CleFin F, CleState* __restrict__ st,
                      int32_t g, float* __restrict__ vsave, int32_t* __restrict__ vtag, int32_t stop_it) {
-    __shared__ CleStepLds L;
+    __shared__ CleStepLds<POS> L;
     __shared__ int flag;
     if (st->done) return;
     int64_t blk = blockIdx.x;
@@ -1255,14 +1279,14 @@
             }
         asm volatile("s_waitcnt vmcnt(0)" ::: "memory");
         __syncthreads();
-        const bool stage_part = (int64_t)F.nl * (F.S + 2) + (int64_t)(sizeof(CleState) / 4) + 2048 <= kCleTile;
+        const bool stage_part = (int64_t)F.nl * (F.S + 2) + (int64_t)(sizeof(CleState) / 4) + kCleFinPart <= kCleFinStack;
         if (F.nl <= 128)
             cle_final_body<true, true>(layers, F.nl, F.part, F.S, F.means, F.hist, st, reinterpret_cast<double*>(lds),
-                                       stage_part ? lds + 2048 : nullptr, nullptr, F.hflag);
+                                       stage_part ? lds + kCleFinPart : nullptr, nullptr, F.hflag);
         else
             cle_final_body<false, true>(layers, F.nl, F.part, F.S, F.means, F.hist, st,
-                                        reinterpret_cast<double*>(lds), stage_part ? lds + 2048 : nullptr,
-                                        lds + kCleTile, F.hflag);
+                                        reinterpret_cast<double*>(lds), stage_part ? lds + kCleFinPart : nullptr,
+                                        lds + kCleFinStack, F.hflag);
 #ifdef DFQ_DIAGNOSTICS
         if (tl2 && threadIdx.x == 0) {
             uint64_t* r = g_cle_tl2 + 4 * kCleTl2Fin;
@@ -1271,6 +1295,8 @@
         }
 #endif
     };
+    bool fin = false;
+    bool stop_block = false;
     if (stop_it >= 0) {
         if (blk < nstop) {
             const int64_t c = blk * (kThreads / 64) + (threadIdx.x >> 6);
@@ -1286,75 +1312,76 @@
             if (threadIdx.x == 0)
                 flag = handoff_arrive(F.cnt + F.nchunks, ((uint32_t)stop_it + 1u) * (uint32_t)nstop - 1u);
             __syncthreads();
-            if (flag) finish();
-            return;
-        }
-        blk -= nstop;
+            fin = flag != 0;
+            stop_block = true;
+        } else {
+            blk -= nstop;
+        }
     }
     const int64_t ntiles = nto + ntp;
-    if (blk >= ntiles) {
+    if (stop_block) {
+    } else if (blk >= ntiles) {
         blk -= ntiles;
         const bool own = blk < nro;
         const int64_t b = own ? blk : blk - nro;
         cle_range_body(rels, rtasks, own ? ro : rp, (own ? ro : rp) + (own ? nro_t : nrp_t), rng, M,
                        own ? (g + 1) & 1 : g & 1, b, own ? nro : nrp, L.tiles);
         tl2_rec(2);
-        return;
-    }
-    const bool own = blk < nto;
-    const int32_t it = own ? g : g - 1;
-    const int64_t tb = own ? blk : blk - nto;
-    const int64_t tnb = own ? nto : ntp;
-    const uint32_t round = (uint32_t)it + 1u;
-    auto arrive = [&](uint32_t* c, uint32_t members) -> bool {
-        asm volatile("s_waitcnt vmcnt(0)" ::: "memory");
-        __syncthreads();
-        if (threadIdx.x == 0) flag = handoff_arrive(c, round * members - 1u);
-        __syncthreads();
-        return flag != 0;
-    };
-    if (F.nbig == 0) {
-        if (own && tb == 0 && F.last) finish();
-        return;
-    }
-    const uint32_t fin_members = (uint32_t)F.nbig;
-    auto hook = [&](const CleUnit& un, const CleChunk& ch, int64_t nb1) {
-        if (!arrive(F.cnt + un.chunk, (uint32_t)(nb1 + 1))) return;
-        {
-            const float* gb1 = b1buf + b1off[un.chunk];
-            const float* gtb = tailbuf + (int64_t)un.chunk * kCleTailWords;
-            const int64_t nw = 32 * nb1;
-            const bool staged = nw + kCleTailWords <= kCleTile;
-            if (staged) {
-                DFQ_LDS float* ll = (DFQ_LDS float*)lds;
-                const DFQ_GLOBAL float* g1 = (const DFQ_GLOBAL float*)gb1;
-                for (int64_t i = threadIdx.x; i < nw; i += kThreads) ll[i] = ld_coh(g1 + i);
-                if (threadIdx.x < kCleTailWords) ll[nw + threadIdx.x] = ld_coh((const DFQ_GLOBAL float*)gtb + threadIdx.x);
-            }
+    } else {
+        const bool own = blk < nto;
+        const int32_t it = own ? g : g - 1;
+        const int64_t tb = own ? blk : blk - nto;
+        const int64_t tnb = own ? nto : ntp;
+        const uint32_t round = (uint32_t)it + 1u;
+        auto arrive = [&](uint32_t* c, uint32_t members) -> bool {
+            asm volatile("s_waitcnt vmcnt(0)" ::: "memory");
             __syncthreads();
-            if (threadIdx.x < 64) {
-                const float fa = staged ? cle_chunk_sum_with(ch, [&](int64_t i) { return lds[i]; },
-                                                             [&](int64_t i) { return lds[nw + i]; }, threadIdx.x)
-                                        : cle_chunk_sum(ch, gb1, gtb, threadIdx.x);
-                if (threadIdx.x == 0) st_coh(F.part + (int64_t)ch.layer * F.S + ch.t, 0.f + fa);
-            }
-        }
-        if (F.stop_arrival && arrive(F.cnt + F.nchunks, fin_members)) finish();
-    };
-    if (F.stop_arrival)
-        cle_tiles_body<decltype(hook)>(layers, chunks, b1off, units + (own ? uo : up), own ? nuo : nup, b1buf, tailbuf,
-                                       tb, tnb, lds, lds + kCleTile + kCleTailWords, hook);
-    else
-        cle_tiles_body(layers, chunks, b1off, units + (own ? uo : up), own ? nuo : nup, b1buf, tailbuf, tb, tnb, lds,
-                       lds + kCleTile + kCleTailWords);
+            if (threadIdx.x == 0) flag = handoff_arrive(c, round * members - 1u);
+            __syncthreads();
+            return flag != 0;
+        };
+        if (F.nbig == 0) {
+            fin = own && tb == 0 && F.last;
+        } else {
+            const uint32_t fin_members = (uint32_t)F.nbig;
+            auto hook = [&](const CleUnit& un, const CleChunk& ch, int64_t nb1) {
+                if (!F.stop_arrival) return;
+                if (!arrive(F.cnt + un.chunk, (uint32_t)(nb1 + 1))) return;
+                {
+                    const float* gb1 = b1buf + b1off[un.chunk];
+                    const float* gtb = tailbuf + (int64_t)un.chunk * kCleTailWords;
+                    const int64_t nw = 32 * nb1;
+                    const bool staged = nw + kCleTailWords <= kCleTailArea;
+                    if (staged) {
+                        DFQ_LDS float* ll = (DFQ_LDS float*)lds;
+                        const DFQ_GLOBAL float* g1 = (const DFQ_GLOBAL float*)gb1;
+                        for (int64_t i = threadIdx.x; i < nw; i += kThreads) ll[i] = ld_coh(g1 + i);
+                        if (threadIdx.x < kCleTailWords)
+                            ll[nw + threadIdx.x] = ld_coh((const DFQ_GLOBAL float*)gtb + threadIdx.x);
+                    }
+                    __syncthreads();
+                    if (threadIdx.x < 64) {
+                        const float fa = staged ? cle_chunk_sum_with(ch, [&](int64_t i) { return lds[i]; },
+                                                                     [&](int64_t i) { return lds[nw + i]; }, threadIdx.x)
+                                                : cle_chunk_sum(ch, gb1, gtb, threadIdx.x);
+                        if (threadIdx.x == 0) st_coh(F.part + (int64_t)ch.layer * F.S + ch.t, 0.f + fa);
+                    }
+                }
+                if (arrive(F.cnt + F.nchunks, fin_members)) fin = true;
+            };
+            cle_tiles_body<decltype(hook)>(layers, chunks, b1off, units + (own ? uo : up), own ? nuo : nup, b1buf, tailbuf,
+                                           tb, tnb, lds, lds + kCleTailArea + kCleTailWords, hook);
 #ifdef DFQ_DIAGNOSTICS
-    if (tl2) {
-        const CleUnit un0 = units[(own ? uo : up) + tb];
-        tl2_rec(un0.tile >= (chunks[un0.chunk].len / 32) / 256 ? 3 : 1);
-    }
+            if (tl2) {
+                const CleUnit un0 = units[(own ? uo : up) + tb];
+                tl2_rec(un0.tile >= (chunks[un0.chunk].len / 32) / 256 ? 3 : 1);
+            }
 #else
-    tl2_rec(1);
+            tl2_rec(1);
 #endif
+        }
+    }
+    if (fin) finish();
 }
 
 __global__ void __launch_bounds__(kThreads)
@@ -2635,6 +2662,8 @@
     return DFQ_OK;
 }
 
+static bool cle_async_join(dfq_cle_plan* p, double seconds = -1.0);
+
 extern "C" int dfq_cle_plan_run(dfq_cle_plan* p, double threshold, int32_t count, int32_t max_iters,
                                 int32_t* iterations, double* diffs, void* stream) {
     if (!p || max_iters < 0 || p->async) return DFQ_ERR_INVALID;
@@ -2644,6 +2673,8 @@
     int dev = 0;
     DFQ_HIP_CHECK(hipGetDevice(&dev));
     CleDeviceCtx& ctx = cle_device_ctx(dev);
+    if (ctx.pending && ctx.pending != p) cle_async_join(ctx.pending);
+    ctx.pending = nullptr;
     std::lock_guard<std::mutex> lock(ctx.mu);
     if (cle_timing()) fprintf(stderr, "DFQ_CLE_TIMING run: caller sync %.1f us, context %.1f us\n", ts1 - ts0,
                               now_us() - ts1);
@@ -2714,7 +2745,7 @@
     return hipSuccess;
 }
 
-static bool cle_async_join(dfq_cle_plan* p, double seconds = -1.0) {
+static bool cle_async_join(dfq_cle_plan* p, double seconds) {
     if (!p || !p->async) return true;
     CleAsync* a = p->async;
     std::unique_lock<std::mutex> l(a->m);
@@ -3068,8 +3099,27 @@
         if (ch.len < 8 || un.tile < 0 || un.tile > ch.len / 32 / 256)
             return fail("unit %lld: tile %lld of chunk %lld", (long long)u, un.tile, un.chunk);
         const int64_t nb1 = ch.len / 32 / 256, e0 = (int64_t)un.tile * kCleTile;
-        if (un.tile < nb1 ? e0 + kCleTile > ch.len : (ch.len - e0 < 0 || ch.len - e0 > kCleTile + kCleTailWords))
+        if (un.tile < nb1 ? e0 + kCleTile > ch.len : (ch.len - e0 < 0 || ch.len - e0 >= kCleTile))
             return fail("unit %lld: tile past chunk %lld (len %lld)", (long long)u, un.chunk, ch.len);
+        if (un.tile == nb1) {
+            const int64_t cnt = ch.len - e0, sz = ch.len / 32, vs = ch.len / 8;
+            const int64_t ni = sz - nb1 * 256, rem_b0 = ni / 16, tail0 = ni % 16;
+            const int64_t npass = cle_tail_passes(rem_b0), per = kCleTailPass / kCleL0Block;
+            for (int64_t ps = 0; ps < npass; ++ps) {
+                const int64_t pc = cle_tail_pass_count(cnt, ps), p0 = ps * kCleTailPass;
+                if (pc < 0 || pc > kCleTailArea || p0 % kCleL0Block != 0)
+                    return fail("unit %lld: tail pass %lld stages %lld elements outside its LDS area", (long long)u, ps, pc);
+                const int64_t mp = std::min(rem_b0 - ps * per, per);
+                int64_t top = kCleL0Block * mp;
+                if (ps == npass - 1) {
+                    top += 32 * tail0;
+                    if (vs > 4 * sz) top = std::max(top, 32 * sz + std::min<int64_t>(24, (vs - 4 * sz) * 8) - e0 - p0);
+                    if (ch.len > 8 * vs) top = std::max(top, ch.len - e0 - p0);
+                }
+                if (mp < 0 || top > pc)
+                    return fail("unit %lld: tail pass %lld reads to word %lld, past what it staged", (long long)u, ps, top);
+            }
+        }
     }
     if ((int32_t)S.uoffs.size() != 2 * NL + 1 || S.uoffs[0] != 0 || S.uoffs.back() != (int64_t)S.units.size())
         return fail("uoffs: %lld entries for %lld launches, last %lld", (long long)S.uoffs.size(), NL, S.uoffs.back());
```

Result: no change. 1931 (median of 3 runs) (-0.7%).
